# lucadellalib/audiocodecs

Measured on AMD Instinct MI355X. Metric: encode+decode audio-sec/s, EnCodec-24k 8cb, higher is better.
Workload: dtype f32 (GEMM-shaped kernels and LSTM products: operands as two scaled fp16 planes, 3 partial products, fp32 accumulate -- split16.h)

## Files before the change

### audiocodecs_amd/csrc/ac_api.hip

```cpp
#include "core.h"
#include "tap_route.h"

extern "C" {

int ac_version(void) { return 400; }

int ac_create(const ac_config* cfg, ac_handle** out) {
    if (!cfg || !out) return AC_EINVAL;
    *out = nullptr;
    if (cfg->struct_size != (int32_t)sizeof(ac_config)) return AC_EINVAL;
    if (cfg->num_ratios < 1 || cfg->num_ratios > AC_MAX_RATIOS || cfg->num_filters < 1 || cfg->hidden_size < 16 ||
        cfg->hidden_size % 16 || cfg->compress < 1 || cfg->num_lstm_layers < 1 || cfg->num_lstm_layers > 2 || cfg->codebook_size % 32 ||
        cfg->codebook_size < 16 || cfg->num_quantizers < 1 || cfg->kernel_size < 1 || cfg->kernel_size > 8 ||
        cfg->last_kernel_size < 1 || cfg->last_kernel_size > 8 || cfg->residual_kernel_size < 1 || cfg->residual_kernel_size > 8)
        return AC_EINVAL;
    int ndev = 0;
    if (hipGetDeviceCount(&ndev) != hipSuccess || ndev <= cfg->device || cfg->device < 0) return AC_ENODEV;
    ac_handle* h = new (std::nothrow) ac_handle();
    if (!h) return AC_ENOMEM;
    h->cfg = *cfg;
    h->hop = 1;
    for (int i = 0; i < cfg->num_ratios; ++i) h->hop *= cfg->upsampling_ratios[i];
    h->D = cfg->num_filters << cfg->num_ratios;
    *out = h;
    return AC_OK;
}







static std::string wavtok_key(const std::string& name) {
    static const std::string pre = "feature_extractor.encodec.encoder.model.";
    if (name.compare(0, pre.size(), pre) != 0) return name;
    std::string k = "encoder.layers." + name.substr(pre.size());
    const size_t cc = k.find(".conv.conv.");
    if (cc != std::string::npos) k = k.substr(0, cc) + ".conv." + k.substr(cc + 11);
    auto ends = [&](const char* sfx) { const size_t n = std::strlen(sfx); return k.size() >= n && k.compare(k.size() - n, n, sfx) == 0; };
    if (ends(".weight_g")) k = k.substr(0, k.size() - 9) + ".parametrizations.weight.original0";
    else if (ends(".weight_v")) k = k.substr(0, k.size() - 9) + ".parametrizations.weight.original1";
    return k;
}

int ac_load_weights(ac_handle* h, const char* name, const void* host_ptr, size_t bytes) {
    if (!h || !name || !host_ptr) return h ? fail(h, AC_EINVAL, "null argument") : AC_EINVAL;
    if (h->finalized) return fail(h, AC_ESTATE, "handle already finalized");
    if (bytes % 4) return fail(h, AC_EINVAL, "tensor '%s': byte size %zu is not a multiple of 4", name, bytes);
    const float* f = static_cast<const float*>(host_ptr);
    h->host[h->arch == ARCH_WAVTOK ? wavtok_key(name) : std::string(name)].assign(f, f + bytes / 4);
    return AC_OK;
}



static void latch_dev_switches(ac_handle* h) {
    auto num = [](const char* name, int dflt) { const char* v = std::getenv(name); return v && *v ? std::atoi(v) : dflt; };
    const char* e = std::getenv("AC_TAP_EPI");
    h->dev.tap_epi_staged = e && std::strcmp(e, "staged") == 0;
    h->dev.tap_dil = num("AC_TAP_DIL", 1);
    h->dev.tap_stagger = num("AC_TAP_STAGGER", 0);
    h->dev.tap_pick = num("AC_TAP_PICK", -1);
    h->dev.tap8 = num("AC_TAP8", -1);
    h->dev.tap8_form = num("AC_TAP8_FORM", 0);
    h->dev.tap8_spread = num("AC_TAP8_SPREAD", 1);
#ifdef AC_DEVELOPER
    h->dev.rb6_dbg = num("AC_RB6_DBG", 0);
    h->dev.lstm_dbg = num("AC_LSTM_DBG", 0);
#endif
    h->dev.rb_stream = num("AC_RB_STREAM", 1);
    h->dev.chain_stream = num("AC_CHAIN_STREAM", 1);
    h->dev.rb128_stream = num("AC_RB128_STREAM", 1);
    h->dev.rb256_fused = num("AC_RB256_FUSED", 1);
    h->dev.front_seg = std::max(0, num("AC_FRONT_SEG", 0));
    h->dev.tail_seg = std::max(0, num("AC_TAIL_SEG", 0));
    h->dev.front_ldspad = std::max(0, num("AC_FRONT_LDSPAD", 0));
    h->dev.lstm_fuse_in = num("AC_LSTM_FUSE_IN", 1);
    const char* r = std::getenv("AC_RVQ");
    h->dev.rvq_exact = r && std::strcmp(r, "fp32") == 0;
    h->dev.prof_detail = num("AC_PROF_DETAIL", 0);
    h->dev.head_seq = num("AC_HEAD_SEQ", 0);
    h->dev.attn_exact = num("AC_ATTN_EXACT", 0);
    h->dev.dac_unit = num("AC_DAC_UNIT", 1);
    h->dev.mimi_tail = num("AC_MIMI_TAIL", 1);
    h->dev.mstream_skinny = num("AC_MSTREAM_SKINNY", -1);
}

int ac_debug_set(ac_handle* h, const char* key, int value) {
    if (!h || !key) return AC_EINVAL;
    struct { const char* k; int* v; } tab[] = {
        {"tap_epi_staged", &h->dev.tap_epi_staged}, {"tap_dil", &h->dev.tap_dil}, {"tap_stagger", &h->dev.tap_stagger}, {"tap_pick", &h->dev.tap_pick}, {"tap8", &h->dev.tap8}, {"tap8_form", &h->dev.tap8_form}, {"tap8_spread", &h->dev.tap8_spread},
        {"rb6_dbg", &h->dev.rb6_dbg}, {"rb_stream", &h->dev.rb_stream}, {"chain_stream", &h->dev.chain_stream}, {"rb128_stream", &h->dev.rb128_stream}, {"rb256_fused", &h->dev.rb256_fused}, {"front_seg", &h->dev.front_seg}, {"tail_seg", &h->dev.tail_seg}, {"front_ldspad", &h->dev.front_ldspad},
        {"lstm_dbg", &h->dev.lstm_dbg}, {"lstm_fuse_in", &h->dev.lstm_fuse_in}, {"rvq_exact", &h->dev.rvq_exact}, {"prof_detail", &h->dev.prof_detail}, {"head_seq", &h->dev.head_seq}, {"attn_exact", &h->dev.attn_exact}, {"dac_unit", &h->dev.dac_unit}, {"mimi_tail", &h->dev.mimi_tail},
        {"mstream_skinny", &h->dev.mstream_skinny},
    };
#ifndef AC_DEVELOPER
    if (std::strcmp(key, "rb6_dbg") == 0 || std::strcmp(key, "lstm_dbg") == 0)
        return fail(h, AC_EINVAL, "ac_debug_set('%s'): a developer-build switch (timing modes with wrong results / fault injection); this is the product library", key);
#endif
    if (!h->finalized) return fail(h, AC_ESTATE, "ac_debug_set('%s'): the switches are latched by ac_finalize; set them afterwards", key);
    for (auto& t : tab)
        if (std::strcmp(t.k, key) == 0) {
            const bool nonneg = t.v == &h->dev.front_seg || t.v == &h->dev.tail_seg || t.v == &h->dev.front_ldspad || t.v == &h->dev.tap_stagger;
            if (nonneg && value < 0) return fail(h, AC_EINVAL, "ac_debug_set('%s', %d): the value must be >= 0", key, value);
            if (t.v == &h->dev.front_ldspad && value > 16384) return fail(h, AC_EINVAL, "ac_debug_set('front_ldspad', %d): at most 16384 bytes", value);
            if (t.v == &h->dev.tap8_form && (value < 0 || value > 5)) return fail(h, AC_EINVAL, "ac_debug_set('tap8_form', %d): 0 (cost model) .. 5", value);
            *t.v = value;
            return AC_OK;
        }
    return fail(h, AC_EINVAL, "ac_debug_set: unknown switch '%s'", key);
}

int ac_set_precision(ac_handle* h, int precision) {
    if (!h) return AC_EINVAL;
    if (h->finalized) return fail(h, AC_ESTATE, "ac_set_precision must precede ac_finalize (weights are packed for one arithmetic)");
    if (precision != AC_PRECISION_FP32 && precision != AC_PRECISION_FP32_EXACT) return fail(h, AC_EINVAL, "unknown precision %d", precision);
    h->precision = precision;
    return AC_OK;
}

int ac_finalize(ac_handle* h) {
    if (!h) return AC_EINVAL;
    if (h->finalized) return fail(h, AC_ESTATE, "handle already finalized");
    {
        int pr = h->precision;
        if (pr < 0) {
            const char* gm = std::getenv("AC_GEMM");
            if (gm && *gm && std::strcmp(gm, "fp32") != 0 && std::strcmp(gm, "split16") != 0)
                return fail(h, AC_EINVAL, "AC_GEMM=%s: unknown arithmetic (fp32 = exact fp32 products, split16 or unset = the default)", gm);
            pr = gm && std::strcmp(gm, "fp32") == 0 ? AC_PRECISION_FP32_EXACT : AC_PRECISION_FP32;
        }
        const char* fz = std::getenv("AC_FUSE");
        h->fuse_chains = !(fz && fz[0] == '0');
        latch_dev_switches(h);
        h->gemm_fp32 = pr == AC_PRECISION_FP32_EXACT;
    }
    if (h->arch == ARCH_MIMI) {
        Packer pk{h};
        if (int rc = mimi_finalize(h, pk)) return rc;
        return upload_blob(h, pk, h->mcfg.device);
    }
    if (h->arch == ARCH_DAC) {
        Packer pk{h};
        if (int rc = dac_finalize(h, pk)) return rc;
        return upload_blob(h, pk, h->dcfg.device);
    }
    if (h->arch == ARCH_WAVTOK) {
        Packer pk{h};
        if (int rc = wavtok_finalize(h, pk)) return rc;
        return upload_blob(h, pk, h->wcfg.device);
    }
    const ac_config& c = h->cfg;
    Arch a = make_arch(c);
    Packer pk{h};
    h->has_enc = h->has_dec = false;
    for (const auto& kv : h->host) {
        if (kv.first.compare(0, 8, "encoder.") == 0) h->has_enc = true;
        if (kv.first.compare(0, 8, "decoder.") == 0) h->has_dec = true;
    }
    if (!h->has_enc && !h->has_dec) return fail(h, AC_ESTATE, "no encoder.* or decoder.* tensor was loaded");
    bool ok = true;
    h->enc_rb.resize(c.num_ratios);
    h->enc_down.resize(c.num_ratios);
    h->dec_up.resize(c.num_ratios);
    h->dec_rb.resize(c.num_ratios);
    if (h->has_enc) {
        ok = pk.conv(a.enc_stem, h->enc_stem);
        for (int i = 0; ok && i < c.num_ratios; ++i) {
            ok = ok && pk.resblock(a.enc_rb3[i], a.enc_rb1[i], a.enc_rbs[i], h->enc_rb[i]);
            ok = ok && pk.conv(a.enc_down[i], h->enc_down[i]);
        }
        ok = ok && pk.lstm(a.enc_lstm, a.D, c.num_lstm_layers, h->enc_lstm);
        ok = ok && pk.conv(a.enc_final, h->enc_final);
        if (ok) pk.chain_bounds(h->enc_stem, h->enc_rb[0], h->enc_down[0], h->enc_front);
// ... 577 lines not shown
```

### audiocodecs_amd/csrc/core.h

```cpp
#pragma once
#include <hip/hip_runtime.h>

#include <algorithm>
#include <cmath>
#include <cstdarg>
#include <cstdio>
#include <cstdlib>
#include <cstring>
#include <map>
#include <string>
#include <vector>

#include "../../include/audiocodecs_amd.h"
#include "lstm_consts.h"
#include "rvq_types.h"
#include "split16.h"
#include "tap_gemm.h"

using namespace ac;

namespace ac {
constexpr int THIN_MAXK = 8;
struct RbFused6Params;
}

namespace acimpl {


struct ConvSpec {
    std::string prefix;
    int transposed, cin, cout, k, s;
};

struct PackedGemm {
    size_t w_off = 0, b_off = 0;
    int N = 0, Ktot = 0;
    bool has_bias = true;
};

struct ResBlockPlan {
    int C;
    PackedGemm c3;
    PackedGemm fused;
    size_t w3f_off = 0, wff_off = 0;
    size_t winv3_off = 0, winvf_off = 0;
    size_t w3p_off = 0, wfp_off = 0;
    float hb0 = 0.f, hb1 = 0.f;
    bool has6 = false;
    bool hb256 = false;
};

struct LstmPlan {
    int D, layers;
    std::vector<PackedGemm> ih;
    std::vector<size_t> hh_off;
    std::vector<size_t> ihpk_off;
    size_t persist_off = 0;
    size_t persist16_off = 0;
    size_t persist16_inv = 0;
    bool has_persist = false;
};

struct MimiTfLayer {
    PackedGemm qkv, o, fc1, fc2;
    size_t ln1_w = 0, ln1_b = 0, ln2_w = 0, ln2_b = 0, sc_a = 0, sc_m = 0;
};

struct MimiPlan {
    PackedGemm enc_stem, enc_final, down, dec_first, dec_head;
    std::vector<ResBlockPlan> enc_rb, dec_rb;
    std::vector<PackedGemm> enc_down, dec_up;
    std::vector<MimiTfLayer> enc_tf, dec_tf;
    size_t up_w = 0;
    PackedGemm in_proj;
    PackedGemm out_proj;
    size_t cb_plain = 0, cb_packed = 0, cb_ee = 0;
    size_t cb16 = 0, cb16_inv = 0;
    size_t rope_cos = 0, rope_sin = 0;
    int rope_T = 0;
    int D = 0;
    struct StreamM { size_t stem_f = 0, stem_inv = 0, head_f = 0, head_inv = 0; float sb0 = 0.f, sb1 = 0.f, fb0 = 0.f, fb1h = 0.f; bool stem_ok = false, head_ok = false; } sm;
};

struct DacResUnitPlan {
    PackedGemm c7, c1;
    size_t a1 = 0, a1i = 0, a2 = 0, a2i = 0;
    int dil = 1;
};

struct DacBlockPlan {
    int C = 0, stride = 1;
    std::vector<DacResUnitPlan> ru;
    size_t a = 0, ai = 0;
    PackedGemm conv;
};

struct DacPlan {
    PackedGemm enc_stem, enc_final, dec_first, dec_head, in_proj0;
    std::vector<DacBlockPlan> enc, dec;
    size_t enc_a = 0, enc_ai = 0, dec_a = 0, dec_ai = 0;
    size_t win = 0, bin = 0, wout = 0, bout = 0, cb = 0, cbn = 0, c2 = 0, proj = 0;
    int H = 0;
};

struct WtResnetPlan {
    size_t n1w = 0, n1b = 0, n2w = 0, n2b = 0;
    PackedGemm c1, c2;
};
struct WtCnxPlan {
    size_t dww = 0, dwb = 0, sc = 0, sh = 0, gamma = 0;
    PackedGemm p1, p2;
};
struct WavtokPlan {
    PackedGemm embed, qkv, proj, head, istft;
    WtResnetPlan rn[4];
    size_t an_w = 0, an_b = 0;
    size_t g5w = 0, g5b = 0;
    size_t nsc = 0, nsh = 0;
    size_t flw = 0, flb = 0;
    size_t w2 = 0;
    std::vector<WtCnxPlan> cnx;
    int bins = 0, npad = 0, hop_pad = 0, taps = 0;
};

struct ProfRec {
    int name_id;
    int count;
    hipEvent_t e0, e1;
    double flops, bytes;
};


}
using namespace acimpl;

enum { ARCH_ENCODEC = 0, ARCH_MIMI = 1, ARCH_DAC = 2, ARCH_WAVTOK = 3 };

struct ac_handle {
    int arch = ARCH_ENCODEC;
    ac_config cfg{};
    ac_mimi_config mcfg{};
    MimiPlan mimi;
    ac_dac_config dcfg{};
    DacPlan dac;
    ac_wavtok_config wcfg{};
    WavtokPlan wt;
    std::string err;
    std::map<std::string, std::vector<float>> host;
    bool finalized = false;
    float* blob = nullptr;
    size_t blob_floats = 0;
    int hop = 1, D = 0;
    PackedGemm enc_stem, enc_final;
    std::vector<ResBlockPlan> enc_rb;
    std::vector<PackedGemm> enc_down;
    LstmPlan enc_lstm, dec_lstm;
    PackedGemm dec_first, dec_head;
    std::vector<PackedGemm> dec_up;
    std::vector<ResBlockPlan> dec_rb;
    size_t cb_plain = 0, cb_packed = 0, cb_ee = 0;
    size_t cb16 = 0, cb16_inv = 0;
    struct ChainBounds { float sb0 = 0.f, sb1 = 0.f, fb0 = 0.f, fb1h = 0.f, fb1x = 0.f; bool ok = false; } enc_front, dec_tail;
    struct StreamImgs { size_t stem_f = 0, stem_inv = 0, down_f = 0, down_inv = 0, up_f = 0, up_inv = 0, head_f = 0, head_inv = 0; bool enc_ok = false, dec_ok = false; } simg;
    struct DevSwitches {
        int tap_epi_staged = 0;
        int tap_dil = 1;
        int tap_stagger = 0;
        int tap_pick = -1;
        int tap8 = -1;
        int tap8_form = 0;
        int tap8_spread = 1;
        int rb6_dbg = 0;
        int rb_stream = 1;
        int rb256_fused = 1;
        int rb128_stream = 1;
        int chain_stream = 1;
        int front_seg = 0, tail_seg = 0;
        int front_ldspad = 0;
        int lstm_dbg = 0;
        int lstm_fuse_in = 1;
        int rvq_exact = 0;
        int prof_detail = 0;
        int attn_exact = 0;
        int dac_unit = 1;
        int mimi_tail = 1;
        int head_seq = 0;
        int mstream_skinny = -1;
    } dev;
    bool fuse_chains = true;
    float* dbg = nullptr;
    size_t dbg_cap = 0, dbg_used = 0;
    std::vector<const void*> lds_opted;
    std::map<size_t, size_t> w6_of;
    std::map<size_t, size_t> t6_of;
    std::map<size_t, size_t> t6inv_of;
    bool noncausal = false;
    bool has_enc = true, has_dec = true;
    bool gemm_fp32 = false;
    std::map<size_t, size_t> winv_of;
    std::map<const void*, int> mimi_streams;
    std::map<const void*, int> mimi_dstreams;
    struct EStreamReg {
        int B;
        std::vector<uint8_t> fresh;
    };
    std::map<const void*, EStreamReg> encodec_streams, encodec_dstreams;
    unsigned* amax_buf = nullptr;
    int amax_B = 0, amax_next = 0;
    unsigned* row_buf = nullptr;
    size_t row_cap = 0, row_next = 0;
    void* own_pool = nullptr;
    size_t own_pool_rows = 0;
    int precision = -1;
    unsigned* lp_ctl = nullptr;
    int num_cus = 0;
    bool lstm_step_only = false;
    unsigned long long* clk_dev = nullptr;
    unsigned* sticky = nullptr;
    unsigned* sticky_dev = nullptr;
    bool prof = false;
    bool prof_detail = false;
    std::vector<ProfRec> recs;
    std::vector<std::string> prof_names;
    std::vector<hipEvent_t> ev_pool;
    size_t ev_used = 0;
};

namespace acimpl {

int fail(ac_handle* h, int code, const char* fmt, ...);


#define HIPCHK(h, call)                                                                         \
    do {                                                                                        \
        hipError_t e_ = (call);                                                                 \
        if (e_ != hipSuccess) return fail(h, AC_EHIP, "%s failed: %s", #call, hipGetErrorString(e_)); \
    } while (0)


inline int cdiv(int a, int b) { return (a + b - 1) / b; }

int ensure_lds(ac_handle* h, const void* func, size_t bytes);

inline size_t align_up(size_t v, size_t a) { return (v + a - 1) / a * a; }


struct Arch {
    std::vector<ConvSpec> enc_rb3, enc_rb1, enc_rbs, enc_down;
    ConvSpec enc_stem, enc_final, dec_first, dec_head;
    std::vector<ConvSpec> dec_up, dec_rb3, dec_rb1, dec_rbs;
    std::string enc_lstm, dec_lstm;
    int D;
};

Arch make_arch(const ac_config& c);


struct Packer {
    ac_handle* h;
    std::vector<float> blob;
    int rc = AC_OK;

    const std::vector<float>* get(const std::string& name, size_t n) {
        auto it = h->host.find(name);
        if (it == h->host.end()) {
            rc = fail(h, AC_ESTATE, "missing tensor '%s'", name.c_str());
            return nullptr;
        }
        if (it->second.size() != n) {
            rc = fail(h, AC_EINVAL, "tensor '%s' has %zu elements, expected %zu", name.c_str(), it->second.size(), n);
            return nullptr;
        }
        return &it->second;
    }
    bool weight(const ConvSpec& s, std::vector<float>& w) {
        const size_t n = (size_t)s.cin * s.cout * s.k;
        auto it = h->host.find(s.prefix + ".weight");
        if (it != h->host.end()) {
            if (it->second.size() != n) {
                rc = fail(h, AC_EINVAL, "tensor '%s.weight' has %zu elements, expected %zu", s.prefix.c_str(), it->second.size(), n);
                return false;
// ... 345 lines not shown
    void tail_bounds(const PackedGemm& up, const ResBlockPlan& rb, const PackedGemm& head, ac_handle::ChainBounds& cb) {
        cb.ok = false;
        if (!use16() || !rb.has6 || !rb.winv3_off || rb.C != 32 || up.N != 64 || up.Ktot != 128 || !h->t6inv_of.count(up.w_off) || head.N != 1 || head.Ktot != 7 * 32) return;
        cb.sb0 = cb.sb1 = 0.f;
        for (int n = 0; n < up.N; ++n) {
            double l1 = 0.0;
            for (int k = 0; k < up.Ktot; ++k) l1 += std::fabs((double)blob[up.w_off + (size_t)n * up.Ktot + k]);
            cb.sb1 = std::max(cb.sb1, (float)(l1 * 1.000001));
            cb.sb0 = std::max(cb.sb0, std::fabs(blob[up.b_off + n]));
        }
        const int hid = rb.C / 2;
        cb.fb0 = cb.fb1h = cb.fb1x = 0.f;
        for (int n = 0; n < rb.C; ++n) {
            double lh = 0.0, lx = 0.0;
            for (int k = 0; k < hid; ++k) lh += std::fabs((double)blob[rb.fused.w_off + (size_t)n * rb.fused.Ktot + k]);
            for (int k = hid; k < rb.fused.Ktot; ++k) lx += std::fabs((double)blob[rb.fused.w_off + (size_t)n * rb.fused.Ktot + k]);
            cb.fb1h = std::max(cb.fb1h, (float)(lh * 1.000001));
            cb.fb1x = std::max(cb.fb1x, (float)(lx * 1.000001));
            cb.fb0 = std::max(cb.fb0, std::fabs(blob[rb.fused.b_off + n]));
        }
        cb.ok = true;
    }
    bool lstm(const std::string& prefix, int D, int layers, LstmPlan& lp) {
        lp.D = D;
        lp.layers = layers;
        for (int l = 0; l < layers; ++l) {
            const std::string sfx = "_l" + std::to_string(l);
            const std::vector<float>* wih = get(prefix + ".weight_ih" + sfx, (size_t)4 * D * D);
            const std::vector<float>* whh = get(prefix + ".weight_hh" + sfx, (size_t)4 * D * D);
            const std::vector<float>* bih = get(prefix + ".bias_ih" + sfx, (size_t)4 * D);
            const std::vector<float>* bhh = get(prefix + ".bias_hh" + sfx, (size_t)4 * D);
            if (!wih || !whh || !bih || !bhh) return false;
            PackedGemm g;
            g.N = 4 * D;
            g.Ktot = D;
            g.w_off = reserve((size_t)4 * D * D);
            std::copy(wih->begin(), wih->end(), blob.begin() + g.w_off);
            g.b_off = reserve((size_t)4 * D);
            for (int n = 0; n < 4 * D; ++n) blob[g.b_off + n] = (*bih)[n] + (*bhh)[n];
            if (l == 0) pack6(g);
            lp.ih.push_back(g);
            const size_t off = reserve((size_t)4 * D * D);
            for (int ug = 0; ug < D / 4; ++ug)
                for (int ks = 0; ks < D / 16; ++ks)
                    for (int lane = 0; lane < 64; ++lane)
                        for (int u = 0; u < 4; ++u) {
                            const int j = lane & 15, kq = lane >> 4;
                            const int row = (j >> 2) * D + ug * 4 + (j & 3);
                            const int k = ks * 16 + 4 * kq + u;
                            blob[off + (((size_t)ug * (D / 16) + ks) * 64 + lane) * 4 + u] = (*whh)[(size_t)row * D + k];
                        }
            lp.hh_off.push_back(off);
            const size_t off2 = reserve((size_t)4 * D * D);
            for (int ug = 0; ug < D / 4; ++ug)
                for (int ks = 0; ks < D / 16; ++ks)
                    for (int lane = 0; lane < 64; ++lane)
                        for (int u = 0; u < 4; ++u) {
                            const int j = lane & 15, kq = lane >> 4;
                            const int row = (j >> 2) * D + ug * 4 + (j & 3);
                            const int k = ks * 16 + 4 * kq + u;
                            blob[off2 + (((size_t)ug * (D / 16) + ks) * 64 + lane) * 4 + u] = (*wih)[(size_t)row * D + k];
                        }
            lp.ihpk_off.push_back(off2);
        }
        if (D == LP_D && layers == 2) {
            const std::vector<float>* mats[3] = {get(prefix + ".weight_hh_l0", (size_t)4 * D * D), get(prefix + ".weight_ih_l1", (size_t)4 * D * D),
                                                 get(prefix + ".weight_hh_l1", (size_t)4 * D * D)};
            const size_t mat = (size_t)LP_SLICES * 4 * 4 * 8 * 256;
            lp.persist_off = reserve(3 * mat);
            for (int m = 0; m < 3; ++m)
                for (int idx = 0; idx < LP_SLICES; ++idx)
                    for (int w = 0; w < 4; ++w)
                        for (int n = 0; n < 4; ++n)
                            for (int ks = 0; ks < 8; ++ks)
                                for (int lane = 0; lane < 64; ++lane)
                                    for (int e = 0; e < 4; ++e)
                                        blob[lp.persist_off + m * mat + ((((size_t)idx * 4 + w) * 4 + n) * 8 + ks) * 256 + lane * 4 + e] =
                                            (*mats[m])[(size_t)(n * D + idx * 16 + (lane & 15)) * D + (w * 8 + ks) * 16 + 4 * (lane >> 4) + e];
            const std::vector<float>* mats6[4] = {mats[0], mats[1], mats[2], get(prefix + ".weight_ih_l0", (size_t)4 * D * D)};
            if (use16()) {
                const size_t mat16 = (size_t)LP_SLICES * 4 * 4 * 4 * 2 * 512;
                lp.persist16_off = reserve((4 * mat16 + 1) / 2);
                lp.persist16_inv = reserve((size_t)2 * 4 * D);
                std::vector<int> sc((size_t)2 * 4 * D);
                const int layer_of[4] = {0, 1, 1, 0};
                for (int l = 0; l < 2; ++l)
                    for (int row = 0; row < 4 * D; ++row) {
                        uint32_t mx = 0;
                        for (int m = 0; m < 4; ++m)
                            if (layer_of[m] == l)
                                for (int k = 0; k < D; ++k) {
                                    uint32_t b;
                                    std::memcpy(&b, &(*mats6[m])[(size_t)row * D + k], 4);
                                    mx = std::max(mx, b & 0x7fffffffu);
                                }
                        sc[(size_t)l * 4 * D + row] = s16_exponent(mx, 40);
                        blob[lp.persist16_inv + (size_t)l * 4 * D + row] = s16_pow2(-sc[(size_t)l * 4 * D + row]);
                    }
                std::vector<uint16_t> pl16(4 * mat16);
                for (int m = 0; m < 4; ++m)
                    for (int idx = 0; idx < LP_SLICES; ++idx)
                        for (int w = 0; w < 4; ++w)
                            for (int n = 0; n < 4; ++n)
                                for (int ks = 0; ks < 4; ++ks)
                                    for (int lane = 0; lane < 64; ++lane)
                                        for (int e = 0; e < 8; ++e) {
                                            const int row = n * D + idx * 16 + (lane & 15);
                                            uint16_t t[3];
                                            split16h((*mats6[m])[(size_t)row * D + w * 128 + ks * 32 + 8 * (lane >> 4) + e], sc[(size_t)layer_of[m] * 4 * D + row], t);
                                            const size_t base = m * mat16 + (((((size_t)idx * 4 + w) * 4 + n) * 4 + ks) * 2) * 512 + (size_t)lane * 8 + e;
                                            pl16[base] = t[0];
                                            pl16[base + 512] = t[1];
                                        }
                std::memcpy(&blob[lp.persist16_off], pl16.data(), pl16.size() * 2);
            }
            lp.has_persist = true;
        }
        return true;
    }
};


struct Act {
    const float* p;
    long long bs, ts;
    int L, C;
    const unsigned* amax = nullptr;
    int amax_n = 0;
};

int prof_name(ac_handle* h, const char* nm);

hipEvent_t next_event(ac_handle* h);


struct ProfScope {
    ac_handle* h;
    hipStream_t st;
    ProfRec r{};
    bool on;
    ProfScope(ac_handle* h_, hipStream_t st_, const char* nm, double flops, double bytes, int count = 1)
        : h(h_), st(st_), on(h_->prof) {
        if (!on) return;
        r.name_id = prof_name(h, nm);
        r.count = count;
        r.flops = flops;
        r.bytes = bytes;
        r.e0 = next_event(h);
        r.e1 = next_event(h);
        (void)hipEventRecord(r.e0, st);
    }
    ~ProfScope() {
        if (!on) return;
        (void)hipEventRecord(r.e1, st);
        h->recs.push_back(r);
    }
};


constexpr int AMAX_SLOTS = 512;

inline size_t pool_bytes(int pool_B, size_t rows) {
    return (size_t)AMAX_SLOTS * std::max(pool_B, 1) * AMAX_STRIDE * 4 + 8 * align_up(std::max<size_t>(rows, 64), 64) * 4 + 256;
}

void pool_bind(ac_handle* h, void* mem, int pool_B, size_t rows);

int amax_begin(ac_handle* h, hipStream_t st, int B);

unsigned* amax_new(ac_handle* h);

const unsigned* amax_of(ac_handle* h, hipStream_t st, const float* x, long long bs, long long ts, int L, int C, int B, const unsigned* known);

unsigned* rowmax_new(ac_handle* h, hipStream_t st, long long rows, bool zero);

const unsigned* amax_plus(ac_handle* h, hipStream_t st, const Act& x, float add, int B);

TapSeg make_seg(const Act& x, int s, int J, int pad , int extra, int kofs, const float* rel_len, int left = -1, int right = 0);


inline bool aligned16(const void* p) { return (reinterpret_cast<uintptr_t>(p) & 15) == 0; }

int run_tap(ac_handle* h, hipStream_t st, TapGemmParams& p);


struct Out {
    float* raw = nullptr;
    float* elu = nullptr;
};

struct Act2 {
    Act raw{}, elu{};
};

int try_thin6(ac_handle* h, hipStream_t st, const PackedGemm& g, const Act& x, int width, int edge, Out out, int B, const unsigned** amax_out = nullptr);

int conv_fwd(ac_handle* h, hipStream_t st, const PackedGemm& g, const Act& x, int k, int s, const float* rel_len, Out out,
             long long out_bs, long long out_rs, int B, Act2* y);

int convtr_fwd(ac_handle* h, hipStream_t st, const PackedGemm& g, const Act& x, int s, Out out, int B, Act2* y);

bool rb128_ok(const ac_handle* h, const ResBlockPlan& rb);

int resblock_fwd(ac_handle* h, hipStream_t st, const ResBlockPlan& rb, const Act2& x, float* hbuf, Out out, int B, Act2* y);
bool rb256_ok(const ac_handle* h, const ResBlockPlan& rb, int L);

bool thin_ok(const ac_config& c, int k);

int thin_stem(ac_handle* h, hipStream_t st, const PackedGemm& g, int F, int k, int pad, const float* sig, const float* rel_len, int B, int T,
              Out out, Act2* y, int padl = -1, const float* alpha = nullptr, const float* alpha_inv = nullptr, int Lp = -1);

int stem_fwd(ac_handle* h, hipStream_t st, const float* sig, const float* rel_len, int B, int T, Out out, Act2* y);

int thin_head(ac_handle* h, hipStream_t st, const PackedGemm& g, int F, int k, int pad, const Act& x, int B, float* sig, int padl = -1,
              int tanh_out = 0);

int head_fwd(ac_handle* h, hipStream_t st, const Act& x, int B, float* sig);

bool enc_front_ok(const ac_handle* h, int T);

int enc_front_fwd(ac_handle* h, hipStream_t st, const float* sig, const float* rel_len, int B, int T, float* y, float* dbg_x0, float* dbg_y1, Act2* out);

bool dec_tail_ok(const ac_handle* h, const Act& xe);

int dec_tail_fwd(ac_handle* h, hipStream_t st, const Act& xe, int B, float* sig, float* dbg_u, float* dbg_v);

void capture(ac_handle* h, hipStream_t st, const Act& a, int B);


struct LstmWs {
    float *gin, *gin1, *hseq0, *hseq1, *c;
};

int lstm_fwd(ac_handle* h, hipStream_t st, const LstmPlan& lp, const Act& x, const LstmWs& ws, Out out, int B, Act2* y);

int rvq_encode_fwd(ac_handle* h, hipStream_t st, const float* feats, int F, int K, long long* toks);

int rvq_decode_fwd(ac_handle* h, hipStream_t st, const long long* toks, int F, int K, float* out);


constexpr int NACT = 6;


struct Workspace {
    size_t act_floats = 0;
    size_t gin = 0, hseq = 0, c = 0;
    int pool_B = 0;
    size_t pool_rows = 0;
    size_t total_bytes = 0;
};

inline void add_pool(Workspace& w, int pool_B, size_t rows) {
    w.pool_B = pool_B;
    w.pool_rows = rows;
    w.total_bytes += pool_bytes(pool_B, rows);
}

Workspace plan_ws(const ac_handle* h, int B, int T_in , int N_frames , bool enc);


struct WsPtrs {
    float* act[NACT];
    bool used[NACT];
    LstmWs lstm;
    float* take() {
        for (int i = 0; i < NACT; ++i)
            if (!used[i]) { used[i] = true; return act[i]; }
        return nullptr;
    }
    void give(const float* p) {
        for (int i = 0; i < NACT; ++i)
            if (act[i] == p) used[i] = false;
    }
    void give(const Act2& a) { give(a.raw.p); give(a.elu.p); }
};

int carve(ac_handle* h, const Workspace& w, void* ws, size_t ws_bytes, WsPtrs* o);

int check_ready(ac_handle* h);

int check_len(ac_handle* h, long long samples);

int encoder_fwd(ac_handle* h, hipStream_t st, const float* sig, const float* rel_len, int B, int T, float* feats, WsPtrs& ws);

int decoder_fwd(ac_handle* h, hipStream_t st, const long long* toks, int B, int N, int K, float* sig, WsPtrs& ws);

bool rb64_identity_head_fwd(ac_handle* h, hipStream_t st, const ResBlockPlan& rb, const Act2& x, const PackedGemm& head, int head_k, float* sig, int B, int* rc);
int enc_stream_fwd(ac_handle* h, hipStream_t st, const float* sig, const float* rel_len, int B, int T, float* y, float* dbg_x0, float* dbg_y1, const unsigned* amax_sig, unsigned* amax_out);
int dec_stream_fwd(ac_handle* h, hipStream_t st, const Act& xe, int B, float* sig, float* dbg_u, float* dbg_v, const unsigned* amax_x);
int launch_rb_stream6m(ac_handle* h, hipStream_t st, const ResBlockPlan& rb, const float* xr, const float* sig, int B, int L, Out out, float* head_y, int head_k,
                       const unsigned* amax_in, unsigned* amax_out);
int launch_rb_stream128m(ac_handle* h, hipStream_t st, RbFused6Params& p, const ResBlockPlan& rb, bool sc, Out out, int B);
int launch_rb_stream6(ac_handle* h, hipStream_t st, RbFused6Params& p, const ResBlockPlan& rb, bool sc, Out out, int B);
int rb64_identity_fwd(ac_handle* h, hipStream_t st, const ResBlockPlan& rb, const Act2& x, Out out, int B, const unsigned** amax_out);
int rb128_identity_fwd(ac_handle* h, hipStream_t st, const ResBlockPlan& rb, const Act2& x, Out out, int B, const unsigned** amax_out);
int rvq_encode_cdist_launch(ac_handle* h, hipStream_t st, const RvqEncParams& p, unsigned blocks, const _Float16* epk16 = nullptr, const float* einv = nullptr);
void rvq_decode_launch(hipStream_t st, const RvqDecParams& p, unsigned blocks);
void amax_fill_launch(hipStream_t st, unsigned* slot, unsigned bits, int B);
int resample_launch(const float* x, int B, int L, const float* kern, int n, int o, int taps, int width, float* y, int L_out, hipStream_t st);
constexpr int RSTREAM_MAX_TAPS = 8192;
long long resample_stream_groups(long long total, int o, int width);
long long resample_stream_out_len(long long consumed, int L, int n, int o, int width, int finish);
size_t resample_stream_state_bytes(int B, int taps);
int resample_stream_reset_launch(void* state, int B, int n, int o, int taps, int width, hipStream_t st);
int resample_stream_push_launch(void* state, const float* x, long long x_pitch, int B, int L, long long consumed, const float* kern, int n, int o, int taps,
                                int width, float* y, long long y_pitch, int m, int finish, hipStream_t st);
int resample_stream_reset_slots_launch(void* state, int B, int n, int o, int taps, int width, const int* slots_dev, int rows, hipStream_t st);
int resample_stream_push_slots_launch(void* state, int B, const int* slots_dev, const long long* consumed_dev, int rows, const float* x, long long x_pitch,
                                      int L, const float* kern, int n, int o, int taps, int width, float* y, long long y_pitch, int m, int finish,
                                      hipStream_t st);

struct Epi {
    const float* scale = nullptr;
    const float* res = nullptr;
    long long res_bs = 0, res_rs = 0;
    int gelu = 0;
    const unsigned* rowmax_in = nullptr;
// ... 32 lines not shown
```

### audiocodecs_amd/csrc/core.hip

```cpp
#include "core.h"
#include "split16_kernels.h"
#include "lstm.h"
#include "lstm_persist.h"
#include "lstm_persist16.h"
#include "rvq.h"
#include "rvq16.h"
#include "tap_gemm4.h"
#include "tap_gemm6.h"
#include "tap_gemm8.h"
#include "tap_route.h"
#include "thin.h"
#include "rb_fused.h"
#include "rb_fused6.h"
#include "thin_conv6.h"
#include "rb_fused6_128.h"
#include "rb256_fused.h"
#include "enc_front.h"
#include "dec_tail.h"

namespace acimpl {


int fail(ac_handle* h, int code, const char* fmt, ...) {
    char buf[1024];
// ... 126 lines not shown
        zero_words(st, r, need);
        if (hipGetLastError() != hipSuccess) return nullptr;
    }
    return r;
}


const unsigned* amax_plus(ac_handle* h, hipStream_t st, const Act& x, float add, int B) {
    if (!x.amax || x.amax_n != B) return nullptr;
    unsigned* slot = amax_new(h);
    if (!slot) return nullptr;
    hipLaunchKernelGGL(amax_add_kernel, dim3(cdiv(B, 64)), dim3(64), 0, st, x.amax, add, slot, B);
    return slot;
}



template <int WGM, int WGN, int WM, int WN>
static int launch_tap(ac_handle* h, hipStream_t st, TapGemmParams p, TapFamily f, const char* name, double flops, double bytes) {
    ProfScope ps(h, st, name, flops, bytes);
    if (f == TapFamily::tap4) {
        using Cfg = Tap4Cfg<WGM, WGN, WM, WN>;
        p.mtiles = cdiv(p.M, Cfg::BM);
        p.ntiles = cdiv(p.N, Cfg::BN);
        if (int rc = ensure_lds(h, reinterpret_cast<const void*>(tap_gemm4_kernel<WGM, WGN, WM, WN>), Cfg::lds_bytes)) return rc;
        const long long blocks = (long long)p.B * p.mtiles * p.ntiles;
        hipLaunchKernelGGL((tap_gemm4_kernel<WGM, WGN, WM, WN>), dim3((unsigned)blocks), dim3(Cfg::NT), Cfg::lds_bytes, st, p);
        return AC_OK;
    }
    constexpr int BM = WGM * WM * 16, BN = WGN * WN * 16;
    p.mtiles = cdiv(p.M, BM);
    p.ntiles = cdiv(p.N, BN);
    const size_t lds = tap_gemm_lds_bytes<WGM, WGN, WM, WN>();
    const long long blocks = (long long)p.B * p.mtiles * p.ntiles;
    if (f == TapFamily::vec) hipLaunchKernelGGL((tap_gemm_kernel<WGM, WGN, WM, WN, true>), dim3((unsigned)blocks), dim3(WGM * WGN * 64), lds, st, p);
    else hipLaunchKernelGGL((tap_gemm_kernel<WGM, WGN, WM, WN, false>), dim3((unsigned)blocks), dim3(WGM * WGN * 64), lds, st, p);
    return AC_OK;
}

static int launch_tap_fp32(ac_handle* h, hipStream_t st, const TapGemmParams& p, const TapRoute& r, const char* name, double flops, double bytes) {
    switch (r.key()) {
    case tap_key(4, 1, 2, 1): return launch_tap<4, 1, 2, 1>(h, st, p, r.family, name, flops, bytes);
    case tap_key(4, 1, 2, 2): return launch_tap<4, 1, 2, 2>(h, st, p, r.family, name, flops, bytes);
    case tap_key(2, 2, 2, 2): return launch_tap<2, 2, 2, 2>(h, st, p, r.family, name, flops, bytes);
    case tap_key(2, 2, 4, 3): return launch_tap<2, 2, 4, 3>(h, st, p, r.family, name, flops, bytes);
    case tap_key(2, 2, 4, 4): return launch_tap<2, 2, 4, 4>(h, st, p, r.family, name, flops, bytes);
    }
    return fail(h, AC_EINVAL, "run_tap: no instantiation of %s", r.name);
}

template <int WGM, int WGN, int WMT, int WN, int HALO>
static int launch_tap6(ac_handle* h, hipStream_t st, TapGemmParams& p, const __bf16* w6, const char* name, double flops, double bytes) {
    using Cfg = Tap6Cfg<WGM, WGN, WMT, WN, HALO>;
    p.mtiles = cdiv(p.M, Cfg::BM);
    p.ntiles = p.N / Cfg::BN;
    const long long blocks = (long long)p.B * p.mtiles * p.ntiles;
    if (int rc = ensure_lds(h, reinterpret_cast<const void*>(tap_gemm6_kernel<WGM, WGN, WMT, WN, 2, HALO>), Cfg::lds_for(2))) return rc;
    ProfScope ps(h, st, name, flops, bytes);
    hipLaunchKernelGGL((tap_gemm6_kernel<WGM, WGN, WMT, WN, 2, HALO>), dim3((unsigned)blocks), dim3(Cfg::NT), Cfg::lds_for(2), st, p, w6);
    return AC_OK;
}

static int launch_tap6_family(ac_handle* h, hipStream_t st, TapGemmParams& p, const TapRoute& r, const __bf16* w6, const char* name, double flops, double bytes) {
    if (r.family == TapFamily::tap6_dil) {
        switch (r.key()) {
        case tap_key(1, 4, 4, 2): return launch_tap6<1, 4, 4, 2, T6_DIL_HALO>(h, st, p, w6, name, flops, bytes);
        case tap_key(1, 4, 4, 1): return launch_tap6<1, 4, 4, 1, T6_DIL_HALO>(h, st, p, w6, name, flops, bytes);
        case tap_key(2, 2, 2, 3): return launch_tap6<2, 2, 2, 3, T6_DIL_HALO>(h, st, p, w6, name, flops, bytes);
        case tap_key(4, 1, 1, 3): return launch_tap6<4, 1, 1, 3, T6_DIL_HALO>(h, st, p, w6, name, flops, bytes);
        }
    } else {
        switch (r.key()) {
        case tap_key(1, 4, 4, 2): return launch_tap6<1, 4, 4, 2, 7>(h, st, p, w6, name, flops, bytes);
        case tap_key(1, 8, 4, 1): return launch_tap6<1, 8, 4, 1, 7>(h, st, p, w6, name, flops, bytes);
        case tap_key(1, 4, 4, 1): return launch_tap6<1, 4, 4, 1, 7>(h, st, p, w6, name, flops, bytes);
        case tap_key(2, 2, 2, 3): return launch_tap6<2, 2, 2, 3, 7>(h, st, p, w6, name, flops, bytes);
        case tap_key(4, 1, 1, 3): return launch_tap6<4, 1, 1, 3, 7>(h, st, p, w6, name, flops, bytes);
        case tap_key(2, 2, 2, 1): return launch_tap6<2, 2, 2, 1, 7>(h, st, p, w6, name, flops, bytes);
        }
    }
    return fail(h, AC_EINVAL, "run_tap: no instantiation of %s", r.name);
}

template <int WGM, int WGN, int WMT, int WN, bool RM, bool J1, bool SP>
static int launch_tap8(ac_handle* h, hipStream_t st, TapGemmParams& p, const __bf16* w6, const char* name, double flops, double bytes) {
    using Cfg = Tap8Cfg<WGM, WGN, WMT, WN>;
    p.mtiles = cdiv(p.M, Cfg::BM);
    p.ntiles = p.N / Cfg::BN;
    const long long blocks = (long long)p.B * p.mtiles * p.ntiles;
    ProfScope ps(h, st, name, flops, bytes);
    if (int rc = ensure_lds(h, reinterpret_cast<const void*>(tap_gemm8_kernel<WGM, WGN, WMT, WN, RM, J1, SP>), Cfg::lds_bytes)) return rc;
    hipLaunchKernelGGL((tap_gemm8_kernel<WGM, WGN, WMT, WN, RM, J1, SP>), dim3((unsigned)blocks), dim3(Cfg::NT), Cfg::lds_bytes, st, p, w6);
    return AC_OK;
}

static int launch_tap8_family(ac_handle* h, hipStream_t st, TapGemmParams& p, const TapRoute& r, const __bf16* w6, const char* name, double flops, double bytes) {
    constexpr int RJ = TK_RM | TK_J1, J = TK_J1, S = TK_SPREAD;
    switch (r.key()) {
    case tap_key(2, 4, 4, 2, RJ): return launch_tap8<2, 4, 4, 2, true, true, false>(h, st, p, w6, name, flops, bytes);
    case tap_key(2, 4, 4, 2, RJ | S): return launch_tap8<2, 4, 4, 2, true, true, true>(h, st, p, w6, name, flops, bytes);
    case tap_key(2, 4, 4, 2, J): return launch_tap8<2, 4, 4, 2, false, true, false>(h, st, p, w6, name, flops, bytes);
    case tap_key(2, 4, 4, 2, J | S): return launch_tap8<2, 4, 4, 2, false, true, true>(h, st, p, w6, name, flops, bytes);
    case tap_key(2, 4, 4, 2): return launch_tap8<2, 4, 4, 2, false, false, false>(h, st, p, w6, name, flops, bytes);
    case tap_key(2, 4, 4, 2, S): return launch_tap8<2, 4, 4, 2, false, false, true>(h, st, p, w6, name, flops, bytes);
    case tap_key(2, 4, 2, 2, RJ): return launch_tap8<2, 4, 2, 2, true, true, false>(h, st, p, w6, name, flops, bytes);
    case tap_key(2, 4, 2, 2, RJ | S): return launch_tap8<2, 4, 2, 2, true, true, true>(h, st, p, w6, name, flops, bytes);
    case tap_key(2, 4, 2, 2, J): return launch_tap8<2, 4, 2, 2, false, true, false>(h, st, p, w6, name, flops, bytes);
    case tap_key(2, 4, 2, 2, J | S): return launch_tap8<2, 4, 2, 2, false, true, true>(h, st, p, w6, name, flops, bytes);
    case tap_key(2, 4, 2, 2): return launch_tap8<2, 4, 2, 2, false, false, false>(h, st, p, w6, name, flops, bytes);
    case tap_key(2, 4, 2, 2, S): return launch_tap8<2, 4, 2, 2, false, false, true>(h, st, p, w6, name, flops, bytes);
    case tap_key(4, 2, 2, 2, RJ): return launch_tap8<4, 2, 2, 2, true, true, false>(h, st, p, w6, name, flops, bytes);
    case tap_key(4, 2, 2, 2, RJ | S): return launch_tap8<4, 2, 2, 2, true, true, true>(h, st, p, w6, name, flops, bytes);
    case tap_key(4, 2, 2, 2, J): return launch_tap8<4, 2, 2, 2, false, true, false>(h, st, p, w6, name, flops, bytes);
    case tap_key(4, 2, 2, 2, J | S): return launch_tap8<4, 2, 2, 2, false, true, true>(h, st, p, w6, name, flops, bytes);
    case tap_key(4, 2, 2, 2): return launch_tap8<4, 2, 2, 2, false, false, false>(h, st, p, w6, name, flops, bytes);
    case tap_key(4, 2, 2, 2, S): return launch_tap8<4, 2, 2, 2, false, false, true>(h, st, p, w6, name, flops, bytes);
    }
    return fail(h, AC_EINVAL, "run_tap: no instantiation of %s", r.name);
}


TapSeg make_seg(const Act& x, int s, int J, int pad , int extra, int kofs, const float* rel_len, int left, int right) {
    TapSeg g{};
    g.x = x.p;
    g.amax = x.amax;
    g.amax_n = x.amax_n;
    g.bs = x.bs;
    g.ts = x.ts;
    g.rel_len = rel_len;
    g.L = x.L;
    g.cin = x.C;
    g.cin_shift = -1;
    for (int sh = 0; sh < 30; ++sh)
        if ((1 << sh) == x.C) g.cin_shift = sh;
    g.s = s;
    g.J = J;
    const int pad_left = left < 0 ? (J - 1) * s : left;
    const int max_pad = std::max(pad_left, right + extra);
    g.Lp = (pad == PAD_REFLECT && x.L <= max_pad) ? max_pad + 1 : x.L;
    g.lim = pad != PAD_ZERO ? x.L + right + extra : x.L;
    g.reflect = pad;
    g.elu = 0;
    g.kofs = kofs;
    g.pad = pad_left;
    g.dil = 1;
    return g;
}


int run_tap(ac_handle* h, hipStream_t st, TapGemmParams& p) {
    const auto w6_it = h->w6_of.find((size_t)(p.w - h->blob));
    const auto iv = h->winv_of.find((size_t)(p.w - h->blob));
    TapRouteInputs in;
    in.w6 = w6_it != h->w6_of.end();
    in.winv = iv != h->winv_of.end();
    in.want_rowmode = p.amax_rows != 0;
    in.want_rows = p.amax_out_rows != nullptr;
    in.gemm_fp32 = h->gemm_fp32;
    const TapRoute r = route_tap(p, in, h->dev);
    if (r.reject_taps) return fail(h, AC_EINVAL, "conv with %d taps exceeds the kernel limit of 8", r.reject_taps);
    double kk = 0, inb = 0;
    for (int i = 0; i < p.nseg; ++i) {
        kk += (double)p.seg[i].J * p.seg[i].s * p.seg[i].cin;
        inb += (double)p.B * p.seg[i].L * p.seg[i].cin * 4.0;
    }
    const double flops = 2.0 * p.B * (double)p.M * p.N * kk;
    const double bytes = inb + (double)p.B * p.M * p.N * 4.0 * ((p.y ? 1 : 0) + (p.y_elu ? 1 : 0)) + (double)p.N * p.Ktot * 4.0;
    std::string name = r.name;
    if (h->prof && h->prof_detail && r.family != TapFamily::scalar && r.family != TapFamily::vec) {
        char shape[64];
        std::snprintf(shape, sizeof shape, " B%d M%d N%d K%d J%d s%d%s", p.B, p.M, p.N, (int)kk, p.seg[0].J, p.seg[0].s, p.seg[0].dil == 1 ? "" : p.seg[0].dil == 3 ? " d3" : " d9");
        name += shape;
    }
    p.amax_out_rows = nullptr;
    p.amax_rows = 0;
    int rc;
    if (r.family == TapFamily::scalar || r.family == TapFamily::vec || r.family == TapFamily::tap4) {
        rc = launch_tap_fp32(h, st, p, r, name.c_str(), flops, bytes);
    } else {
        p.clk = h->clk_dev;
#ifdef T6_TRACE
        if (const char* ts = std::getenv("AC_TRACE_SHAPE")) {
            int tm = 0, tn = 0, tk = 0;
            if (std::sscanf(ts, "%d,%d,%d", &tm, &tn, &tk) == 3 && !((tm == 0 || tm == p.M) && tn == p.N && tk == (int)kk)) p.clk = nullptr;
        }
#endif
        if (r.rowmode) {
            TapSeg& sg = p.seg[0];
            if (!(sg.amax && sg.amax_n == -p.M)) {
                unsigned* rm = rowmax_new(h, st, p.M, false);
                if (!rm) return fail(h, AC_ENOMEM, "the workspace pool's row ring is too small for %d rows", p.M);
                ProfScope ps(h, st, "rowmax_kernel", 0.0, (double)p.M * sg.cin * 4.0);
                hipLaunchKernelGGL(rowmax_kernel, dim3((unsigned)cdiv(p.M, 4)), dim3(256), 0, st, sg.x, sg.ts, (long long)p.M, sg.cin, rm);
                sg.amax = rm;
            }
            p.amax_rows = 1;
            p.winv = h->blob + iv->second;
            if (r.rows_out) {
                p.amax_out_rows = rowmax_new(h, st, p.M, true);
                if (!p.amax_out_rows) return fail(h, AC_ENOMEM, "the workspace pool's row ring is too small for %d rows", p.M);
            }
        } else if (in.winv) {
            for (int i = 0; i < p.nseg; ++i) {
                TapSeg& sg = p.seg[i];
                sg.amax = amax_of(h, st, sg.x, sg.bs, sg.ts, sg.L, sg.cin, p.B, sg.amax_n == p.B ? sg.amax : nullptr);
                if (!sg.amax) return fail(h, AC_ESTATE, "out of amax slots (split16.h)");
            }
            p.winv = h->blob + iv->second;
            p.amax_out = amax_new(h);
            p.epi_direct = r.epi_direct;
        }
        p.stagger = h->dev.tap_stagger;
        const __bf16* w6 = reinterpret_cast<const __bf16*>(h->blob + w6_it->second);
        rc = r.family == TapFamily::tap8 ? launch_tap8_family(h, st, p, r, w6, name.c_str(), flops, bytes)
                                         : launch_tap6_family(h, st, p, r, w6, name.c_str(), flops, bytes);
    }
    if (rc) return rc;
    HIPCHK(h, hipGetLastError());
    return AC_OK;
}


int try_thin6(ac_handle* h, hipStream_t st, const PackedGemm& g, const Act& x, int width, int edge, Out out, int B, const unsigned** amax_out) {
    if (h->gemm_fp32 || g.N != 64 || g.Ktot != 128 || x.C != width || x.ts != width || x.bs != (long long)x.L * width ||
        (x.L * width) % 64 || x.L * width < 256 || !aligned16(x.p) || (long long)x.L * width * 4 > 0x70000000LL)
        return 1;
    auto it = h->t6_of.find(g.w_off);
    if (it == h->t6_of.end()) return 1;
    ThinConv6Params p{};
    p.x = x.p;
    p.wf = reinterpret_cast<const __bf16*>(h->blob + it->second);
    p.bias = h->blob + g.b_off;
    p.y = out.raw;
    p.y_elu = out.elu;
    p.B = B;
    p.Ls = x.L * width / 64;
    p.M = p.Ls;
    p.ntiles = cdiv(p.M, T6_BM);
    p.edge = edge;
    const bool s16 = h->t6inv_of.count(g.w_off) != 0;
    if (s16) {
        p.amax_in = amax_of(h, st, x.p, x.bs, x.ts, x.L, x.C, B, x.amax_n == B ? x.amax : nullptr);
        if (!p.amax_in) return fail(h, AC_ESTATE, "out of amax slots (split16.h)");
        p.winv = h->blob + h->t6inv_of[g.w_off];
        p.amax_out = amax_new(h);
        if (amax_out) *amax_out = p.amax_out;
    }
    const long long total = (long long)B * p.ntiles;
    const int grid = (int)std::min<long long>(total, 4 * 256);
    ProfScope ps(h, st, "thin_conv6_kernel<2>", 2.0 * B * p.M * 64.0 * 128.0,
                 (double)B * p.M * 256.0 * (1 + (out.raw ? 1 : 0) + (out.elu ? 1 : 0)));
    hipLaunchKernelGGL(thin_conv6_kernel<2>, dim3(grid), dim3(256), T6_LDS, st, p);
    return AC_OK;
}


int conv_fwd(ac_handle* h, hipStream_t st, const PackedGemm& g, const Act& x, int k, int s, const float* rel_len, Out out,
             long long out_bs, long long out_rs, int B, Act2* y) {
    const int M = cdiv(x.L, s);
    const int extra = M * s - x.L;
    if (s == 2 && k == 4 && !rel_len && extra == 0 && x.L >= 4 && out_rs == 64 && out_bs == (long long)M * 64 && !h->noncausal) {
        const unsigned* am = nullptr;
        const int rc = try_thin6(h, st, g, x, 32, 1, out, B, &am);
        if (rc <= 0) {
            if (y && !rc) {
                y->raw = Act{out.raw, out_bs, out_rs, M, g.N, am, B};
                y->elu = Act{out.elu, out_bs, out_rs, M, g.N, am, B};
            }
            if (!rc) HIPCHK(h, hipGetLastError());
            return rc;
        }
    }
    TapGemmParams p{};
    p.nseg = 1;
    if (s != 1 && k != 2 * s) return fail(h, AC_EINVAL, "strided conv needs kernel == 2*stride (got k=%d, s=%d)", k, s);
    if (h->noncausal) {
        const int total = k - s, right = total / 2;
        p.seg[0] = make_seg(x, s, s == 1 ? k : 2, PAD_REFLECT, extra, 0, rel_len, total - right, right);
    } else {
        p.seg[0] = make_seg(x, s, s == 1 ? k : 2, PAD_REFLECT, extra, 0, rel_len);
    }
    p.w = h->blob + g.w_off;
    p.bias = g.has_bias ? h->blob + g.b_off : nullptr;
    p.y = out.raw;
    p.y_elu = out.elu;
    p.y_bs = out_bs;
    p.y_rs = out_rs;
    p.B = B;
    p.M = M;
    p.N = g.N;
    p.Ktot = g.Ktot;
    const int rc = run_tap(h, st, p);
    if (y) {
        y->raw = Act{out.raw, out_bs, out_rs, M, g.N, p.amax_out, p.B};
        y->elu = Act{out.elu, out_bs, out_rs, M, g.N, p.amax_out, p.B};
    }
    return rc;
}


int convtr_fwd(ac_handle* h, hipStream_t st, const PackedGemm& g, const Act& x, int s, Out out, int B, Act2* y) {
    const int cout = g.N / s;
    if (s == 2) {
        const unsigned* am = nullptr;
        const int rc = try_thin6(h, st, g, x, 64, 0, out, B, &am);
        if (rc <= 0) {
            if (!rc) {
                y->raw = Act{out.raw, (long long)x.L * s * cout, cout, x.L * s, cout, am, B};
                y->elu = Act{out.elu, (long long)x.L * s * cout, cout, x.L * s, cout, am, B};
                HIPCHK(h, hipGetLastError());
            }
            return rc;
        }
    }
    TapGemmParams p{};
    p.nseg = 1;
    p.seg[0] = make_seg(x, 1, 2, PAD_ZERO, 0, 0, nullptr);
    p.w = h->blob + g.w_off;
    p.bias = h->blob + g.b_off;
    p.y = out.raw;
    p.y_elu = out.elu;
    p.y_bs = (long long)x.L * g.N;
    p.y_rs = g.N;
    p.B = B;
    p.M = x.L;
    p.N = g.N;
    p.Ktot = g.Ktot;
    const int rc = run_tap(h, st, p);
    y->raw = Act{out.raw, (long long)x.L * s * cout, cout, x.L * s, cout, p.amax_out, p.B};
    y->elu = Act{out.elu, (long long)x.L * s * cout, cout, x.L * s, cout, p.amax_out, p.B};
    return rc;
}


template <int C, int BM, int NSPLIT, bool SC = true>
int launch_rb_fused(ac_handle* h, hipStream_t st, const ResBlockPlan& rb, const Act2& x, Out out, int B, int pad = PAD_REFLECT) {
    using Cfg = RbCfg<C, BM, NSPLIT, SC>;
    RbFusedParams p{};
    p.xe = x.elu.p;
    p.xr = x.raw.p;
    p.w3 = h->blob + rb.c3.w_off;
    p.b3 = h->blob + rb.c3.b_off;
    p.wf = h->blob + rb.fused.w_off;
    p.bf = h->blob + rb.fused.b_off;
    p.y = out.raw;
    p.y_elu = out.elu;
    p.B = B;
    p.L = x.raw.L;
    p.Lp = x.raw.L > 2 ? x.raw.L : 3;
    p.ntiles = cdiv(x.raw.L, BM);
    p.pad = pad;
    if (int rc = ensure_lds(h, reinterpret_cast<const void*>(rb_fused_kernel<C, BM, NSPLIT, SC>), Cfg::lds_bytes)) return rc;
    const long long total = (long long)B * p.ntiles;
    const int grid = (int)std::min<long long>(total, 512);
    const size_t lds = Cfg::lds_bytes;
    const double L = x.raw.L;
    ProfScope ps(h, st, !SC ? "rb_fused_kernel<64, 64, 2, false>" : C == 32 ? "rb_fused_kernel<32, 128, 1>" : "rb_fused_kernel<64, 64, 2>",
                 2.0 * B * L * ((double)(C / 2) * 3 * C + (double)C * Cfg::KF),
                 (double)B * L * C * 4.0 * ((x.elu.p ? 2 : 1) + (out.raw ? 1 : 0) + (out.elu ? 1 : 0)));
    hipLaunchKernelGGL((rb_fused_kernel<C, BM, NSPLIT, SC>), dim3(grid), dim3(256), lds, st, p);
    return AC_OK;
}


bool rb_split16(ac_handle* h, hipStream_t st, const ResBlockPlan& rb, const Act2& x, int B, RbFused6Params& p, const unsigned** amax_out) {
    if (h->gemm_fp32 || !rb.winv3_off) return false;
    p.amax_in = amax_of(h, st, x.raw.p, x.raw.bs, x.raw.ts, x.raw.L, x.raw.C, B, x.raw.amax_n == B ? x.raw.amax : nullptr);
    p.winv3 = h->blob + rb.winv3_off;
    p.winvf = h->blob + rb.winvf_off;
    p.hb0 = rb.hb0;
    p.hb1 = rb.hb1;
    p.amax_out = amax_new(h);
    if (amax_out) *amax_out = p.amax_out;
    return true;
}


template <int C, bool SC>
int launch_rb_fused6(ac_handle* h, hipStream_t st, const ResBlockPlan& rb, const Act2& x, Out out, int B, int pad = PAD_REFLECT, const unsigned** amax_out = nullptr,
                     const PackedGemm* head = nullptr, int head_k = 0, float* head_y = nullptr) {
    using Cfg = Rb6Cfg<C, SC>;
    RbFused6Params p{};
    const bool with_head = head && C == 64 && !SC;
    if (with_head) {
        p.head_w = h->blob + head->w_off;
        p.head_b = h->blob + head->b_off;
        p.head_y = head_y;
        p.head_k = head_k;
    }
    p.xr = x.raw.p;
    p.w3f = reinterpret_cast<const __bf16*>(h->blob + rb.w3f_off);
    p.wff = reinterpret_cast<const __bf16*>(h->blob + rb.wff_off);
    p.b3 = h->blob + rb.c3.b_off;
    p.bf = h->blob + rb.fused.b_off;
    p.y = out.raw;
    p.y_elu = out.elu;
    p.B = B;
    p.L = x.raw.L;
    p.lpad = h->noncausal ? 1 : 2;
    p.Lp = x.raw.L > p.lpad ? x.raw.L : p.lpad + 1;
    p.ntiles = cdiv(x.raw.L, with_head ? Cfg::BM - (head_k - 1) : Cfg::BM);
    p.pad = pad;
    p.dbg = h->dev.rb6_dbg;
    if (!rb_split16(h, st, rb, x, B, p, amax_out)) return fail(h, AC_ESTATE, "fused residual block without split16 images");
    if (!p.amax_in) return fail(h, AC_ESTATE, "out of amax slots (split16.h)");
    if (with_head) p.amax_out = nullptr;
    const double L = x.raw.L;
    if (C == 64 && !with_head && h->dev.rb_stream && p.lpad == 2 && rb.w3p_off && (long long)x.raw.L * 256 < 0x70000000LL)
        return launch_rb_stream6(h, st, p, rb, SC, out, B);
    const size_t lds6 = with_head ? Cfg::lds_bytes16_head : Cfg::lds_bytes16;
// ... 295 lines not shown
        return AC_OK;
    }
    size_t lds = EF_LDS;
    lds += (size_t)h->dev.front_ldspad;
    if (int rc = ensure_lds(h, reinterpret_cast<const void*>(enc_front_kernel), lds)) return rc;
    const long long streams = (long long)B * p.segs_per_clip;
    {
        ProfScope ps(h, st, "enc_front_kernel", 2.0 * B * (double)T * (7.0 * 32 + 16.0 * 96 + 32.0 * 48 + 64.0 * 128 / 2),
                     (double)B * T * 4.0 + (double)B * p.M * 256.0);
        hipLaunchKernelGGL(enc_front_kernel, dim3((unsigned)cdiv((int)streams, EF_WAVES)), dim3(64 * EF_WAVES), lds, st, p);
    }
    HIPCHK(h, hipGetLastError());
    out->raw = Act{y, (long long)p.M * 64, 64, p.M, 64, p.amax_out, B};
    out->elu = Act{nullptr, (long long)p.M * 64, 64, p.M, 64, p.amax_out, B};
    return AC_OK;
}


bool dec_tail_ok(const ac_handle* h, const Act& xe) {
    const ac_config& c = h->cfg;
    return h->fuse_chains && h->arch == ARCH_ENCODEC && !h->noncausal && !h->gemm_fp32 && h->dec_tail.ok &&
           c.num_filters == 32 && c.last_kernel_size == 7 && c.residual_kernel_size == 3 && c.compress == 2 && c.num_ratios >= 1 &&
           c.upsampling_ratios[c.num_ratios - 1] == 2 && xe.p && xe.C == 64 && xe.ts == 64 && xe.bs == (long long)xe.L * 64 && aligned16(xe.p) &&
           xe.L >= 32 && (long long)xe.L * 256 < 0x70000000LL;
}


int dec_tail_fwd(ac_handle* h, hipStream_t st, const Act& xe, int B, float* sig, float* dbg_u, float* dbg_v) {
    const int last = h->cfg.num_ratios - 1;
    const ResBlockPlan& rb = h->dec_rb[last];
    const PackedGemm& gu = h->dec_up[last];
    DecTailParams p{};
    p.xe = xe.p;
    p.wuf = reinterpret_cast<const __bf16*>(h->blob + h->t6_of[gu.w_off]);
    p.w3f = reinterpret_cast<const __bf16*>(h->blob + rb.w3f_off);
    p.wff = reinterpret_cast<const __bf16*>(h->blob + rb.wff_off);
    p.bu = h->blob + gu.b_off;
    p.winvu = h->blob + h->t6inv_of[gu.w_off];
    p.b3 = h->blob + rb.c3.b_off;
    p.winv3 = h->blob + rb.winv3_off;
    p.bf = h->blob + rb.fused.b_off;
    p.winvf = h->blob + rb.winvf_off;
    p.wh = h->blob + h->dec_head.w_off;
    p.bh = h->blob + h->dec_head.b_off;
    p.sig = sig;
    p.dbg_u = dbg_u;
    p.dbg_v = dbg_v;
    p.B = B;
    p.L = xe.L;
    const int nchunks = cdiv(xe.L, DT_ROWS);
    p.seg_chunks = std::max(8, cdiv(nchunks, std::max(1, 6144 / B)));
    if (h->dev.tail_seg > 0) p.seg_chunks = h->dev.tail_seg;
    p.segs_per_clip = cdiv(nchunks, p.seg_chunks);
    p.amax_x = amax_of(h, st, xe.p, xe.bs, xe.ts, xe.L, xe.C, B, xe.amax_n == B ? xe.amax : nullptr);
    if (!p.amax_x) return fail(h, AC_ESTATE, "out of amax slots (split16.h)");
    p.ub0 = h->dec_tail.sb0; p.ub1 = h->dec_tail.sb1;
    p.hb0 = rb.hb0; p.hb1 = rb.hb1;
    if (h->dev.chain_stream && h->simg.dec_ok) {
        if (int rc = dec_stream_fwd(h, st, xe, B, sig, dbg_u, dbg_v, p.amax_x)) return rc;
        HIPCHK(h, hipGetLastError());
        return AC_OK;
    }
    if (int rc = ensure_lds(h, reinterpret_cast<const void*>(dec_tail_kernel), DT_LDS)) return rc;
    const long long streams = (long long)B * p.segs_per_clip;
    {
        ProfScope ps(h, st, "dec_tail_kernel", 2.0 * B * (double)xe.L * (64.0 * 128 + 2.0 * (16.0 * 96 + 32.0 * 48 + 7.0 * 32)),
                     (double)B * xe.L * 256.0 + (double)B * xe.L * 8.0);
        hipLaunchKernelGGL(dec_tail_kernel, dim3((unsigned)cdiv((int)streams, 8)), dim3(512), DT_LDS, st, p);
    }
    HIPCHK(h, hipGetLastError());
    return AC_OK;
}


void capture(ac_handle* h, hipStream_t st, const Act& a, int B) {
    if (!h->dbg) return;
    const size_t n = (size_t)B * a.L * a.C;
    if (h->dbg_used + n <= h->dbg_cap)
        (void)hipMemcpyAsync(h->dbg + h->dbg_used, a.p, n * sizeof(float), hipMemcpyDeviceToDevice, st);
    h->dbg_used += n;
}


int lstm_fwd(ac_handle* h, hipStream_t st, const LstmPlan& lp, const Act& x, const LstmWs& ws, Out out, int B, Act2* y) {
    const int D = lp.D, T = x.L, L = lp.layers;
    if (D % 64 != 0 || D > 512) return fail(h, AC_EINVAL, "LSTM width %d unsupported (need 64, 128, 256 or 512)", D);
    if (L < 1 || L > 2) return fail(h, AC_EINVAL, "%d LSTM layers unsupported (1 or 2)", L);
    hipStreamCaptureStatus cap = hipStreamCaptureStatusNone;
    (void)hipStreamIsCapturing(st, &cap);
    const bool persist = lp.has_persist && h->lp_ctl && h->num_cus == 256 && !h->lstm_step_only && x.ts == D && cap == hipStreamCaptureStatusNone;
    const bool fuse_env = h->dev.lstm_fuse_in != 0;
    const bool fuse_in = persist && !h->gemm_fp32 && fuse_env && aligned16(x.p) && x.bs % 4 == 0;
    if (!fuse_in) {
        TapGemmParams p{};
        p.nseg = 1;
        p.seg[0] = make_seg(x, 1, 1, PAD_ZERO, 0, 0, nullptr);
        p.w = h->blob + lp.ih[0].w_off;
        p.bias = h->blob + lp.ih[0].b_off;
        p.y = ws.gin;
        p.y_bs = 4LL * D;
        p.y_rs = (long long)B * 4 * D;
        p.B = B;
        p.M = T;
        p.N = 4 * D;
        p.Ktot = D;
        int rc = run_tap(h, st, p);
        if (rc) return rc;
    }
    const int nroles = 2 * L - 1, nlaunch = T + 2 * (L - 1);
    const long long BD = (long long)((B + 31) / 32 * 32) * D, B4D = (long long)B * 4 * D;
    if (persist) {
        const int chunks = cdiv(B, 64);
        const unsigned* x_amax = nullptr;
        if (fuse_in && lp.persist16_inv) {
            x_amax = amax_of(h, st, x.p, x.bs, x.ts, x.L, x.C, B, x.amax_n == B ? x.amax : nullptr);
            if (!x_amax) return fail(h, AC_ESTATE, "out of amax slots (split16.h)");
        }
        int* poison = reinterpret_cast<int*>(ws.c);
        if (!h->gemm_fp32) HIPCHK(h, hipMemsetAsync(poison, 0x7f, (size_t)B * sizeof(int), st));
        ProfScope ps(h, st, h->gemm_fp32 ? "lstm_persist_kernel" : fuse_in ? "lstm_persist16_kernel<true>" : "lstm_persist16_kernel<false>", 2.0 * T * (double)B * 4 * D * D * (nroles + (fuse_in ? 1 : 0)),
                     (double)T * ((double)B * 4 * D * 4 + 3.0 * B * D * 4) + 12.0 * D * D * 4, chunks);
        auto tail = [&](int c0, int nb, const int* pz) {
            LstmTailParams tp{};
            tp.ctl = h->lp_ctl;
            tp.sticky = h->sticky_dev;
            tp.poison = pz;
            tp.yout = out.raw;
            tp.yout_elu = out.elu;
            tp.y_bs = (long long)T * D;
            tp.clip0 = c0;
            tp.B = nb;
            tp.T = T;
            tp.D = D;
            tp.xcds_used = 8;
            hipLaunchKernelGGL(lstm_tail_kernel, dim3(nb, 4), dim3(256), 0, st, tp);
        };
        for (int c0 = 0; c0 < B; c0 += 64) {
            LstmPersistParams q{};
            q.gin0 = ws.gin;
            q.w_pk = h->blob + lp.persist_off;
            q.bias1 = h->blob + lp.ih[1].b_off;
            q.hseq0 = ws.hseq0;
            q.hseq1 = ws.hseq1;
            q.skip = x.p;
            q.yout = out.raw;
            q.yout_elu = out.elu;
            q.ctl = h->lp_ctl;
            q.gin_ts = B4D;
            q.h_ts = BD;
            q.skip_bs = x.bs;
            q.y_bs = (long long)T * D;
            q.B = std::min(64, B - c0);
            q.T = T;
            q.group0 = c0 / 16;
            q.clip0 = c0;
            q.dbg = h->dev.lstm_dbg;
            if (!h->gemm_fp32) {
                LstmPersist16Params q6{};
                q6.base = q;
                q6.base.h_ts = (long long)((B + 31) / 32 * 2) * LP16_GROUP_BYTES;
                q6.winv = h->blob + lp.persist16_inv;
                q6.amax_x = fuse_in ? x_amax : nullptr;
                q6.w_pk6 = reinterpret_cast<const __bf16*>(h->blob + lp.persist16_off);
                q6.bias0 = h->blob + lp.ih[0].b_off;
                q6.fuse_in = fuse_in ? 1 : 0;
                q6.poison = poison;
                q6.hseq0_local = ws.gin1;
                HIPCHK(h, hipMemsetAsync(h->lp_ctl, 0, LP_CTL_WORDS * sizeof(unsigned), st));
                const size_t hbytes = (size_t)T * (size_t)q6.base.h_ts;
                const size_t rbytes = (size_t)std::min(T, LP16_RING) * (size_t)q6.base.h_ts;
                HIPCHK(h, hipMemsetAsync(ws.hseq0, 0xFF, hbytes, st));
                HIPCHK(h, hipMemsetAsync(ws.hseq1, 0xFF, rbytes, st));
                HIPCHK(h, hipMemsetAsync(ws.gin1, 0xFF, rbytes, st));
                void* args6[] = {&q6};
                const void* kfn = fuse_in ? reinterpret_cast<const void*>(lstm_persist16_kernel<true>) : reinterpret_cast<const void*>(lstm_persist16_kernel<false>);
                HIPCHK(h, hipLaunchCooperativeKernel(kfn, dim3(256), dim3(512), args6, 0, st));
                tail(c0, q.B, poison);
                if (AC_DEV_MODE(q.dbg, 32)) {
                    HIPCHK(h, hipStreamSynchronize(st));
                    std::vector<unsigned long long> tr(8 * 64);
                    HIPCHK(h, hipMemcpy(tr.data(), h->lp_ctl + LP_CTL_FLAGS, tr.size() * 8, hipMemcpyDeviceToHost));
                    for (int role = 0; role < 2; ++role) {
                        std::fprintf(stderr, "lstm trace role %d (layer %d), 10 ns units from step start: ", role, role & 1);
                        for (int s_ = 0; s_ < 4; ++s_) {
                            const unsigned long long* r = &tr[role * 64 + s_ * 8];
                            std::fprintf(stderr, "| t=%d:", 100 + s_);
                            for (int k = 1; k < 8; ++k) std::fprintf(stderr, " %lld", r[k] ? (long long)(r[k] - r[0]) : -1LL);
                            if (s_ < 3) std::fprintf(stderr, " next %lld ", (long long)(r[8] - r[0]));
                        }
                        const double us3 = (double)(tr[role * 64 + 24] - tr[role * 64]) * 0.01;
                        std::fprintf(stderr, " | steps that had to poll: %llu of %d | shader clock %.0f MHz\n", tr[role * 64 + 63], T,
                                     us3 > 0 ? (double)(tr[role * 64 + 33] - tr[role * 64 + 32]) / us3 : 0.0);
                    }
                }
                continue;
            }
            HIPCHK(h, hipMemsetAsync(h->lp_ctl, 0, LP_CTL_WORDS * sizeof(unsigned), st));
            void* args[] = {&q};
            HIPCHK(h, hipLaunchCooperativeKernel(reinterpret_cast<const void*>(lstm_persist_kernel), dim3(256), dim3(256), args, 0, st));
            tail(c0, q.B, nullptr);
        }
        HIPCHK(h, hipGetLastError());
        const unsigned* am = amax_plus(h, st, x, 1.0f, B);
        y->raw = Act{out.raw, (long long)T * D, D, T, D, am, B};
        y->elu = Act{out.elu, (long long)T * D, D, T, D, am, B};
        return AC_OK;
    }
    {
        ProfScope ps(h, st, "lstm_step_kernel", 2.0 * T * (double)B * 4 * D * D * nroles,
                     (double)T * nroles * ((double)B * 4 * D * 4 + 4.0 * D * D * 4 + 2.0 * B * D * 4), nlaunch);
        for (int s = 0; s < nlaunch; ++s) {
            LstmLaunchParams q{};
            q.B = B;
            q.D = D;
            auto fill_last = [&](LstmRole& r, int t) {
                r.skip = x.p + (long long)t * x.ts;
                r.skip_bs = x.bs;
                r.yout = out.raw ? out.raw + (long long)t * D : nullptr;
                r.yout_elu = out.elu ? out.elu + (long long)t * D : nullptr;
                r.y_bs = (long long)T * D;
            };
            {
                LstmRole& r = q.role[0];
                r.active = s < T;
                r.kind = 0;
                r.a = s > 0 ? ws.hseq0 + (long long)(s - 1) * BD : nullptr;
                r.wpk = h->blob + lp.hh_off[0];
                r.gin = ws.gin + (long long)s * B4D;
                r.hnext = ws.hseq0 + (long long)s * BD;
                r.c = ws.c;
                r.first = s == 0;
                if (L == 1 && r.active) fill_last(r, s);
            }
            if (L == 2) {
                const int t1 = s - 1, t2 = s - 2;
                LstmRole& pr = q.role[1];
                pr.active = t1 >= 0 && t1 < T;
                pr.kind = 1;
                pr.a = ws.hseq0 + (long long)std::max(t1, 0) * BD;
                pr.wpk = h->blob + lp.ihpk_off[1];
                pr.bias = h->blob + lp.ih[1].b_off;
                pr.gout = ws.gin1 + (long long)std::max(t1, 0) * B4D;
                LstmRole& r = q.role[2];
                r.active = t2 >= 0 && t2 < T;
                r.kind = 0;
                r.a = t2 > 0 ? ws.hseq1 + (long long)(t2 - 1) * BD : nullptr;
                r.wpk = h->blob + lp.hh_off[1];
                r.gin = ws.gin1 + (long long)std::max(t2, 0) * B4D;
                r.hnext = ws.hseq1 + (long long)std::max(t2, 0) * BD;
                r.c = ws.c + (long long)B * D;
                r.first = t2 == 0;
                if (r.active) fill_last(r, t2);
            }
            const dim3 grid(D / 4, cdiv(B, 32), nroles), block(256);
            switch (D / 32) {
                case 2: hipLaunchKernelGGL(lstm_step_kernel<2>, grid, block, 0, st, q); break;
                case 4: hipLaunchKernelGGL(lstm_step_kernel<4>, grid, block, 0, st, q); break;
                case 8: hipLaunchKernelGGL(lstm_step_kernel<8>, grid, block, 0, st, q); break;
                default: hipLaunchKernelGGL(lstm_step_kernel<16>, grid, block, 0, st, q); break;
            }
        }
    }
    HIPCHK(h, hipGetLastError());
    const unsigned* am = amax_plus(h, st, x, 1.0f, B);
    y->raw = Act{out.raw, (long long)T * D, D, T, D, am, B};
    y->elu = Act{out.elu, (long long)T * D, D, T, D, am, B};
    return AC_OK;
}


int rvq_encode_fwd(ac_handle* h, hipStream_t st, const float* feats, int F, int K, long long* toks) {
    RvqEncParams p{};
    p.x = feats;
    p.epk = h->blob + h->cb_packed;
    p.e = h->blob + h->cb_plain;
    p.ee = h->blob + h->cb_ee;
    p.toks = toks;
    p.F = F;
    p.H = h->cfg.hidden_size;
    p.C = h->cfg.codebook_size;
    p.K = K;
    p.xs = p.H;
    p.tK = K;
    p.tk0 = 0;
    const int HV = p.H / 16;
    const int MS = (HV <= 8 && F >= 1024 * 32) ? 3 : 1;
    const dim3 grid(cdiv(F, 16 * MS)), block(64);
    const bool exact_env = h->dev.rvq_exact != 0;
// ... 113 lines not shown
    if (h->sticky) {
        volatile unsigned* s = h->sticky;
        const unsigned a = s[ST_LSTM_TIMEOUT], b = s[ST_LSTM_PLACEMENT], t = s[ST_BAD_TOKEN];
        if (a || b || t) {
            s[ST_LSTM_TIMEOUT] = 0;
            s[ST_LSTM_PLACEMENT] = 0;
            s[ST_BAD_TOKEN] = 0;
            char lstm[400] = "", tok[200] = "";
            if (a || b) {
                h->lstm_step_only = true;
                std::snprintf(lstm, sizeof lstm,
                              "an EARLIER call's persistent LSTM launch failed (%u bounded waits expired, %u launches without 32 workgroups on "
                              "every XCD -- is the GPU shared?): that call's outputs were set to NaN; the handle now uses the per-step LSTM "
                              "kernels, repeat the call", a, b);
            }
            if (t) std::snprintf(tok, sizeof tok, "an EARLIER ac_decode / ac_dequantize call got %u token ids outside [0, codebook_size): those frames were set to NaN", t);
            return fail(h, (a || b) ? AC_EHIP : AC_EINVAL, "%s%s%s", lstm, (a || b) && t ? "; ALSO: " : "", tok);
        }
    }
    return AC_OK;
}


int check_len(ac_handle* h, long long samples) {
    const long long lim = 0x70000000LL / (h->arch == ARCH_DAC ? 512 : 256) - 1;
    if (samples > lim) return fail(h, AC_EINVAL, "clip of %lld samples is too long for one call (limit %lld): split it", samples, lim);
    return AC_OK;
}


int encoder_fwd(ac_handle* h, hipStream_t st, const float* sig, const float* rel_len, int B, int T, float* feats, WsPtrs& ws) {
    const ac_config& c = h->cfg;
    const bool dbg = h->dbg != nullptr;
    Act xin{sig, (long long)T, 1, T, 1};
    Act2 x, y;
    int rc;
    auto rb_self_elu = [&](int C) {
        if (h->noncausal && h->gemm_fp32) return false;
        return (C == 32 || C == 64 || (C == 128 && c.num_ratios > 2 && rb128_ok(h, h->enc_rb[2]))) && c.residual_kernel_size == 3 && c.compress == 2;
    };
    auto rb256_self_elu = [&](int i, int L) { return i < c.num_ratios && h->enc_rb[i].C == h->enc_down[i - 1].N && rb256_ok(h, h->enc_rb[i], L); };
    int i0 = 0;
    if (enc_front_ok(h, T)) {
        float* d0 = dbg ? ws.take() : nullptr;
        float* d1 = dbg ? ws.take() : nullptr;
        rc = enc_front_fwd(h, st, sig, rel_len, B, T, ws.take(), d0, d1, &x);
        if (rc) return rc;
        if (dbg) {
            capture(h, st, Act{d0, (long long)T * 32, 32, T, 32}, B);
            capture(h, st, Act{d1, (long long)T * 32, 32, T, 32}, B);
            ws.give(d0);
            ws.give(d1);
        }
        capture(h, st, x.raw, B);
        i0 = 1;
    } else {
    if (thin_ok(c, c.kernel_size))
        rc = stem_fwd(h, st, sig, rel_len, B, T, Out{ws.take(), rb_self_elu(c.num_filters) ? nullptr : ws.take()}, &x);
    else
        rc = conv_fwd(h, st, h->enc_stem, xin, c.kernel_size, 1, rel_len, Out{ws.take(), ws.take()},
                      (long long)T * c.num_filters, c.num_filters, B, &x);
    if (rc) return rc;
    capture(h, st, x.raw, B);
    }
    for (int i = i0; i < c.num_ratios; ++i) {
        const int ratio = c.upsampling_ratios[c.num_ratios - 1 - i];
        float* hb = ws.take();
        rc = resblock_fwd(h, st, h->enc_rb[i], x, hb, Out{dbg ? ws.take() : nullptr, ws.take()}, B, &y);
        if (rc) return rc;
        ws.give(hb);
        ws.give(x);
        if (dbg) { capture(h, st, y.raw, B); ws.give(y.raw.p); y.raw.p = nullptr; }
        x = y;
        const int M = cdiv(x.elu.L, ratio);
        const bool last = i == c.num_ratios - 1;
        rc = conv_fwd(h, st, h->enc_down[i], x.elu, 2 * ratio, ratio, nullptr,
                      Out{ws.take(), (last || rb_self_elu(h->enc_down[i].N) || rb256_self_elu(i + 1, M)) ? nullptr : ws.take()},
                      (long long)M * h->enc_down[i].N, h->enc_down[i].N, B, &y);
        if (rc) return rc;
        ws.give(x);
        x = y;
        capture(h, st, x.raw, B);
    }
    rc = lstm_fwd(h, st, h->enc_lstm, x.raw, ws.lstm, Out{dbg ? ws.take() : nullptr, ws.take()}, B, &y);
    if (rc) return rc;
    ws.give(x);
    if (dbg) { capture(h, st, y.raw, B); ws.give(y.raw.p); y.raw.p = nullptr; }
    x = y;
    rc = conv_fwd(h, st, h->enc_final, x.elu, c.last_kernel_size, 1, nullptr, Out{feats, nullptr},
                  (long long)x.elu.L * c.hidden_size, c.hidden_size, B, nullptr);
    ws.give(x);
    return rc;
}


int decoder_fwd(ac_handle* h, hipStream_t st, const long long* toks, int B, int N, int K, float* sig, WsPtrs& ws) {
    const ac_config& c = h->cfg;
    const bool dbg = h->dbg != nullptr;
    float* zb = ws.take();
    int rc = rvq_decode_fwd(h, st, toks, B * N, K, zb);
    if (rc) return rc;
    Act z{zb, (long long)N * c.hidden_size, c.hidden_size, N, c.hidden_size};
    Act2 x, y;
    rc = conv_fwd(h, st, h->dec_first, z, c.kernel_size, 1, nullptr, Out{ws.take(), nullptr}, (long long)N * h->D, h->D, B, &x);
    if (rc) return rc;
    ws.give(zb);
    capture(h, st, x.raw, B);
    rc = lstm_fwd(h, st, h->dec_lstm, x.raw, ws.lstm, Out{dbg ? ws.take() : nullptr, ws.take()}, B, &y);
    if (rc) return rc;
    ws.give(x);
    if (dbg) { capture(h, st, y.raw, B); ws.give(y.raw.p); y.raw.p = nullptr; }
    x = y;
    for (int i = 0; i < c.num_ratios; ++i) {
        if (i == c.num_ratios - 1 && dec_tail_ok(h, x.elu)) {
            const long long T2 = 2LL * x.elu.L;
            float* d0 = dbg ? ws.take() : nullptr;
            float* d1 = dbg ? ws.take() : nullptr;
            rc = dec_tail_fwd(h, st, x.elu, B, sig, d0, d1);
            if (rc) return rc;
            if (dbg) {
                capture(h, st, Act{d0, T2 * 32, 32, (int)T2, 32}, B);
                capture(h, st, Act{d1, T2 * 32, 32, (int)T2, 32}, B);
                ws.give(d0);
                ws.give(d1);
            }
            ws.give(x);
            return AC_OK;
        }
        const int cup = h->dec_up[i].N / c.upsampling_ratios[i];
        const bool self_elu = ((cup == 32 || cup == 64 || (cup == 128 && rb128_ok(h, h->dec_rb[i]))) && c.residual_kernel_size == 3 &&
                               c.compress == 2) ||
                              (cup == h->dec_rb[i].C && rb256_ok(h, h->dec_rb[i], x.elu.L * c.upsampling_ratios[i]));
        rc = convtr_fwd(h, st, h->dec_up[i], x.elu, c.upsampling_ratios[i], Out{ws.take(), self_elu ? nullptr : ws.take()}, B, &y);
        if (rc) return rc;
        ws.give(x);
        x = y;
        capture(h, st, x.raw, B);
        float* hb = ws.take();
        rc = resblock_fwd(h, st, h->dec_rb[i], x, hb, Out{dbg ? ws.take() : nullptr, ws.take()}, B, &y);
        if (rc) return rc;
        ws.give(hb);
        ws.give(x);
        if (dbg) { capture(h, st, y.raw, B); ws.give(y.raw.p); y.raw.p = nullptr; }
        x = y;
    }
    if (thin_ok(c, c.last_kernel_size) && x.elu.ts == c.num_filters)
        rc = head_fwd(h, st, x.elu, B, sig);
    else
        rc = conv_fwd(h, st, h->dec_head, x.elu, c.last_kernel_size, 1, nullptr, Out{sig, nullptr}, (long long)x.elu.L, 1, B, nullptr);
    ws.give(x);
    return rc;
}

int mimi_linear(ac_handle* h, hipStream_t st, const PackedGemm& g, const float* x, long long rows, int cin, int x_pitch, int kofs,
                float* y, int y_pitch, const Epi& epi) {
    const long long widest = std::max<long long>(std::max(x_pitch, y_pitch), g.N);
    long long chunk = ((1LL << 31) / 4 - 4096) / widest / 128 * 128;
    if (chunk < 128) return fail(h, AC_EINVAL, "linear layer too wide for the tap-GEMM (%lld)", widest);
    for (long long r0 = 0; r0 < rows; r0 += chunk) {
        const long long n = std::min(chunk, rows - r0);
        TapGemmParams p{};
        p.nseg = 1;
        Act xa{x + r0 * x_pitch, 0, x_pitch, (int)n, cin};
        const bool one = r0 == 0 && n == rows;
        if (one && epi.rowmax_in) { xa.amax = epi.rowmax_in; xa.amax_n = -(int)n; }
        p.seg[0] = make_seg(xa, 1, 1, PAD_ZERO, 0, kofs, nullptr);
        if (one && epi.rowmax_out) p.amax_out_rows = reinterpret_cast<unsigned*>(1);
        p.amax_rows = 1;
        p.w = h->blob + g.w_off;
        p.bias = g.has_bias ? h->blob + g.b_off : nullptr;
        p.y = y + r0 * y_pitch;
        p.y_bs = 0;
        p.y_rs = y_pitch;
        p.B = 1;
        p.M = (int)n;
        p.N = g.N;
        p.Ktot = g.Ktot;
        p.scale = epi.scale;
        p.res = epi.res ? epi.res + r0 * epi.res_rs : nullptr;
        p.res_bs = 0;
        p.res_rs = epi.res_rs;
        p.gelu = epi.gelu;
        if (int rc = run_tap(h, st, p)) return rc;
        if (epi.rowmax_out) *epi.rowmax_out = one ? p.amax_out_rows : nullptr;
    }
    return AC_OK;
}

int upload_blob(ac_handle* h, Packer& pk, int device) {
    HIPCHK(h, hipSetDevice(device));
    hipDeviceProp_t prop;
// ... 126 lines not shown
```

### audiocodecs_amd/csrc/lstm_persist.h

```cpp
#pragma once
#include "lstm_consts.h"
#include <hip/hip_runtime.h>
#include "lstm.h"

namespace ac {


struct LstmPersistParams {
    const float* gin0;
    const float* w_pk;
    const float* bias1;
    float* hseq0;
    float* hseq1;
    const float* skip;
    float* yout;
    float* yout_elu;
    unsigned* ctl;
    long long gin_ts, h_ts, skip_bs, y_bs;
    int B, T;
    int group0;
    int clip0;
    int dbg;
};

constexpr int LP_CTL_SLOTS = 0;
constexpr int LP_CTL_TIMEOUT = 8 * 16;
constexpr int LP_CTL_FLAGS = 9 * 16;
constexpr int LP_CTL_WORDS = LP_CTL_FLAGS + 4 * 2 * LP_SLICES * LP_FLAG_STRIDE;

typedef unsigned u32x4_lp __attribute__((ext_vector_type(4)));
#define LP_RLX __ATOMIC_RELAXED, __HIP_MEMORY_SCOPE_AGENT
constexpr int LP_SC1 = 16;
constexpr int LP_SC0 = 1;

__device__ __forceinline__ unsigned lp_xcc_id() { return __builtin_amdgcn_s_getreg((3 << 11) | 20) & 0xf; }

__global__ __launch_bounds__(256) void lstm_persist_probe_kernel(unsigned* hist) {
    if (threadIdx.x == 0) atomicAdd(&hist[lp_xcc_id() & 15], 1u);
}

constexpr int LP_NEVER = 0x7f7f7f7f;

struct LstmTailParams {
    const unsigned* ctl;
    unsigned* sticky;
    const int* poison;
    float* yout;
    float* yout_elu;
    long long y_bs;
    int clip0, B, T, D;
    int xcds_used;
};

__global__ __launch_bounds__(256) void lstm_tail_kernel(const LstmTailParams p) {
    const int b = blockIdx.x;
    const unsigned tmo = p.ctl[LP_CTL_TIMEOUT];
    bool placed = true;
    for (int x = 0; x < 8; ++x) {
        const unsigned n = p.ctl[LP_CTL_SLOTS + x * 16];
        placed = placed && (x < p.xcds_used ? n == 32u : n <= 32u);
    }
    const bool failed = tmo != 0u || !placed;
    if (failed && b == 0 && blockIdx.y == 0 && threadIdx.x == 0)
        __hip_atomic_fetch_add(&p.sticky[(tmo == 2u || !placed) ? ST_LSTM_PLACEMENT : ST_LSTM_TIMEOUT], 1u, __ATOMIC_RELAXED, __HIP_MEMORY_SCOPE_SYSTEM);
    int t0 = p.T;
    if (failed) t0 = 0;
    else if (p.poison) {
        const int q = p.poison[p.clip0 + b];
        if (q < p.T) {
            t0 = q;
            if (blockIdx.y == 0 && threadIdx.x == 0)
                __hip_atomic_fetch_add(&p.sticky[ST_NONFINITE_CLIPS], 1u, __ATOMIC_RELAXED, __HIP_MEMORY_SCOPE_SYSTEM);
        }
    }
    if (t0 >= p.T) return;
    const float nan = __uint_as_float(0x7fc00000u);
    const long long n = (long long)(p.T - t0) * p.D;
    const long long o = (long long)(p.clip0 + b) * p.y_bs + (long long)t0 * p.D;
    for (long long i = (long long)blockIdx.y * 256 + threadIdx.x; i < n; i += 256LL * gridDim.y) {
        if (p.yout) p.yout[o + i] = nan;
        if (p.yout_elu) p.yout_elu[o + i] = nan;
    }
}

__device__ __forceinline__ bool lp_wait(unsigned* flags, unsigned want, unsigned* tmo, int lane, int dbg = 0) {
    if (AC_DEV_MODE(dbg, 4)) return true;
    for (unsigned spins = 0;; ++spins) {
        const unsigned f = lane < LP_SLICES ? __hip_atomic_load(&flags[lane * LP_FLAG_STRIDE], LP_RLX) : 0xffffffffu;
        if (__all(f >= want)) return true;
        if ((spins & 1023) == 1023 && __hip_atomic_load(tmo, LP_RLX)) return false;
        if (spins > (1u << 22)) { __hip_atomic_store(tmo, 1u, LP_RLX); return false; }
    }
}

__global__ __launch_bounds__(256) void lstm_persist_kernel(const LstmPersistParams p) {
    constexpr int D = LP_D;
    __shared__ float part[4][4][16][17];
    __shared__ unsigned s_x, s_slot;
    __shared__ int s_okp, s_okr;
    const int tid = threadIdx.x, lane = tid & 63, wave = tid >> 6;
    const int li = lane & 15, kq = lane >> 4;
    unsigned* tmo = p.ctl + LP_CTL_TIMEOUT;
    if (tid == 0) {
        s_x = lp_xcc_id();
        s_slot = __hip_atomic_fetch_add(&p.ctl[LP_CTL_SLOTS + (s_x & 7) * 16], 1u, LP_RLX);
    }
    __syncthreads();
    const int x = s_x & 7, slot = s_slot;
    const int g = x >> 1;
    const int G = (p.B + 15) >> 4;
    if (slot >= 32) {
        if (tid == 0) __hip_atomic_store(tmo, 2u, LP_RLX);
        return;
    }
    if (g >= G) return;
    if (AC_DEV_MODE(p.dbg, 1) && (slot >> 4) == 1) return;
    const int layer = slot >> 4, idx = (x & 1) * 16 + (slot & 15), u0 = idx * 16;

    f32x4 wa[4][8], wb[4][8];
    {
        const long long mat = (long long)LP_SLICES * 4 * 4 * 8 * 256;
        const float* base = p.w_pk + ((long long)idx * 4 + wave) * (4 * 8 * 256) + lane * 4;
        const float* pa = base + (layer == 0 ? 0 : mat);
        const float* pb = base + 2 * mat;
#pragma unroll
        for (int n = 0; n < 4; ++n)
#pragma unroll
            for (int ks = 0; ks < 8; ++ks) {
                wa[n][ks] = *reinterpret_cast<const f32x4*>(pa + (n * 8 + ks) * 256);
                wb[n][ks] = layer ? *reinterpret_cast<const f32x4*>(pb + (n * 8 + ks) * 256) : f32x4{0.f, 0.f, 0.f, 0.f};
            }
    }
    unsigned* flags0 = p.ctl + LP_CTL_FLAGS + ((g * 2 + 0) * LP_SLICES) * LP_FLAG_STRIDE;
    unsigned* flags1 = p.ctl + LP_CTL_FLAGS + ((g * 2 + 1) * LP_SLICES) * LP_FLAG_STRIDE;
    unsigned* myflag = (layer ? flags1 : flags0) + idx * LP_FLAG_STRIDE;
    float* hmine = layer ? p.hseq1 : p.hseq0;
    const long long goff = (long long)(p.group0 + g) * (D / 16) * 256;

    const int ec = tid >> 4, ej = tid & 15;
    const int eb = g * 16 + ec;
    const bool live = eb < p.B;
    const long long erow = (long long)(p.clip0 + eb);
    const int eu = u0 + ej;
    float cstate = 0.f;
    float bq[4] = {0.f, 0.f, 0.f, 0.f};
    if (layer == 1) {
#pragma unroll
        for (int q = 0; q < 4; ++q) bq[q] = p.bias1[q * D + eu];
    }
    const int hpos = (((ej >> 2) << 4) + ec) * 4 + (ej & 3);

    auto load_a = [&](const float* seq, int t, f32x4 (&a)[8]) {
        const float* src = seq + (long long)t * p.h_ts + goff + (long long)(wave * 8) * 256;
        const __amdgpu_buffer_rsrc_t rs = __builtin_amdgcn_make_buffer_rsrc((void*)src, 0, 8 * 1024, 0x00020000);
#pragma unroll
        for (int ks = 0; ks < 8; ++ks) a[ks] = __builtin_bit_cast(f32x4, __builtin_amdgcn_raw_buffer_load_b128(rs, (ks * 64 + lane) * 16, 0, LP_SC1));
    };
    f32x4 accP[4];
    auto project = [&](int t) -> bool {
        if (wave == 0) { const bool ok = lp_wait(flags0, (unsigned)(t + 1), tmo, lane, p.dbg); if (lane == 0) s_okp = ok; }
        __syncthreads();
        if (!s_okp) return false;
        f32x4 a[8];
        load_a(p.hseq0, t, a);
// ... 86 lines not shown
```

### audiocodecs_amd/csrc/lstm_persist16.h

```cpp
#pragma once
#include "lstm_persist.h"
#include "tap_gemm6.h"
#include "rb_fused6.h"
#include <type_traits>

namespace ac {

constexpr int LP16_SLICE_BYTES = 2 * 16 * 16 * 2;
constexpr long long LP16_GROUP_BYTES = (long long)LP_SLICES * LP16_SLICE_BYTES;
#ifndef LP16_RING_N
#define LP16_RING_N 8
#endif
constexpr int LP16_RING = LP16_RING_N;
static_assert(LP16_RING >= 4 && (LP16_RING & (LP16_RING - 1)) == 0, "ring of the recurrent exchange: a power of two, >= 4 (see above)");

struct LstmPersist16Params {
    LstmPersistParams base;
    const __bf16* w_pk6;
    const float* bias0;
    int fuse_in;
    int* poison;
    const float* winv;
    const unsigned* amax_x;
    void* hseq0_local;
// ... 145 lines not shown
    };
    auto load_valid = [&](const char* seq, int t, bf16x8 (&a)[2][2]) -> bool {
        for (unsigned spins = 0;; ++spins) {
            load_a(seq, t, a);
            if (valid(a) || AC_DEV_MODE(p.dbg, 4)) return true;
            if ((spins & 63) == 63 && __hip_atomic_load(tmo, LP_RLX)) return false;
            if (spins > (1u << 18)) { __hip_atomic_store(tmo, 1u, LP_RLX); return false; }
            __builtin_amdgcn_s_sleep(4);
        }
    };
    bf16x8 arec[2][2];
    float skip_next = 0.f;
    f32x4 accP[4];
    const bool xlive = g * 16 + li < p.B;
    const __amdgpu_buffer_rsrc_t xrs = __builtin_amdgcn_make_buffer_rsrc(
        (void*)(p.skip + (long long)(p.clip0 + g * 16) * p.skip_bs), 0, (int)(((long long)(p.B - g * 16 < 16 ? p.B - g * 16 : 16)) * p.skip_bs * 4), 0x00020000);
    const int xoff = xlive ? (int)((long long)li * p.skip_bs * 4) + (wave * 64 + 8 * kq) * 4 : 0x7fff0000;
    f32x4 xr[2][2];
    auto fetch0 = [&](int t) {
#pragma unroll
        for (int ks = 0; ks < 2; ++ks)
#pragma unroll
            for (int hf = 0; hf < 2; ++hf)
                xr[ks][hf] = bufload16(xrs, xlive ? xoff + (t * D + ks * 32 + hf * 4) * 4 : 0x7fff0000, 0);
    };
    float xsc = 1.f, xcr[4] = {1.f, 1.f, 1.f, 1.f};
    if (fuse0) {
        const int cb = p.clip0 + g * 16, cl = p.clip0 + p.B - 1;
        xsc = s16_pow2(s16_exponent(*amax_at(pp.amax_x, cb + li <= cl ? cb + li : cl)));
#pragma unroll
        for (int r = 0; r < 4; ++r) xcr[r] = s16_pow2(LP16_HEXP - s16_exponent(*amax_at(pp.amax_x, cb + kq * 4 + r <= cl ? cb + kq * 4 + r : cl)));
    }
    bf16x8 xa[2][2];
    auto convert0 = [&]() {
        bf16x8 (&a)[2][2] = xa;
#pragma unroll
        for (int ks = 0; ks < 2; ++ks) {
            typedef _Float16 f16x4v __attribute__((ext_vector_type(4)));
            const f32x4 s0 = xr[ks][0] * xsc, s1 = xr[ks][1] * xsc;
            const f16x4v h0 = __builtin_convertvector(s0, f16x4v), h1 = __builtin_convertvector(s1, f16x4v);
            const f16x4v l0 = __builtin_convertvector(s0 - __builtin_convertvector(h0, f32x4), f16x4v);
            const f16x4v l1 = __builtin_convertvector(s1 - __builtin_convertvector(h1, f32x4), f16x4v);
            a[ks][0] = __builtin_bit_cast(bf16x8, __builtin_shufflevector(h0, h1, 0, 1, 2, 3, 4, 5, 6, 7));
            a[ks][1] = __builtin_bit_cast(bf16x8, __builtin_shufflevector(l0, l1, 0, 1, 2, 3, 4, 5, 6, 7));
        }
    };
    auto project0 = [&](int t, int trec, auto rec_tag) {
        bf16x8 (&a)[2][2] = xa;
#pragma unroll
        for (int n = 0; n < 4; ++n) accP[n] = f32x4{0.f, 0.f, 0.f, 0.f};
        if constexpr (decltype(rec_tag)::value && !LATE) load_a(hmine, rt(trec), arec);
        mac(a, wb, accP, 0, 1);
        mac(a, wb, accP, 1, 2);
#pragma unroll
        for (int n = 0; n < 4; ++n)
#pragma unroll
            for (int r = 0; r < 4; ++r) accP[n][r] *= xcr[r];
        if constexpr (decltype(rec_tag)::value && LATE) {
            __builtin_amdgcn_sched_barrier(0);
            await_publish(trec);
            load_a(hmine, rt(trec), arec);
        }
        (void)t;
    };
    auto project = [&](int t) -> bool {
        bf16x8 a[2][2];
        if (!load_valid(h0b, t, a)) return false;
#pragma unroll
        for (int n = 0; n < 4; ++n) accP[n] = f32x4{0.f, 0.f, 0.f, 0.f};
        mac(a, wa, accP);
        return true;
    };
#pragma unroll
    for (int n = 0; n < 4; ++n) accP[n] = f32x4{0.f, 0.f, 0.f, 0.f};
    if (layer == 1 && !project(0)) return;
    if (fuse0) {
        fetch0(0);
        convert0();
        project0(0, 0, std::false_type{});
        fetch0(p.T > 1 ? 1 : 0);
    }
    const float* skip_row = p.skip + (live ? erow : (long long)p.clip0) * p.skip_bs + eu;
    if (layer == 1) skip_next = skip_row[0];
    bf16x8 ap[2][2];
    if (layer == 1) load_a(h0b, p.T > 1 ? 1 : 0, ap);

    const bool trc = AC_DEV_MODE(p.dbg, 32) && idx == 0 && tid == 0;
    unsigned long long* trw = reinterpret_cast<unsigned long long*>(p.ctl + LP_CTL_FLAGS) + (g * 2 + layer) * 64;
#define LP16_TRC(pt_) do { if (trc && t >= 100 && t < 104) trw[(t - 100) * 8 + (pt_)] = __builtin_amdgcn_s_memrealtime(); } while (0)
    auto step = [&](int t) -> bool {
        if (trc && t >= 100 && t < 104) { trw[(t - 100) * 8 + 6] = 0; trw[(t - 100) * 8 + 7] = 0; }
        LP16_TRC(0);
        if (trc && (t == 100 || t == 103)) trw[32 + (t == 103)] = __builtin_amdgcn_s_memtime();
        float gpre[4] = {bq[0], bq[1], bq[2], bq[3]};
        const float skipv = skip_next;
        if (live && layer == 0 && !FUSE) {
            const float* gp = p.gin0 + (long long)t * p.gin_ts + erow * (4 * D);
#pragma unroll
            for (int q = 0; q < 4; ++q) gpre[q] = gp[q * D + eu];
        }
        f32x4 acc[4];
#pragma unroll
        for (int n = 0; n < 4; ++n) acc[n] = accP[n];
        if (t > 0) {
            const bool first_ok = (layer == 1 || fuse0) && (valid(arec) || AC_DEV_MODE(p.dbg, 4));
            if (trc && !first_ok) trw[63] += 1;
            if (!first_ok && !load_valid(hmine, rt(t - 1), arec)) return false;
            LP16_TRC(1);
            if (layer == 0) mac(arec, wa, acc);
            else mac(arec, wb, acc);
        }
        bool ap_ok = true;
        if (fuse0) {
            convert0();
            fetch0(t + 2 < p.T ? t + 2 : p.T - 1);
        }
        if (layer == 1) ap_ok = valid(ap) || AC_DEV_MODE(p.dbg, 4);
        LP16_TRC(2);
        f32x4 (&pt)[8][16][LP16_PART_PITCH] = part[t & 1];
#pragma unroll
        for (int r = 0; r < 4; ++r) pt[wave][kq * 4 + r][li] = f32x4{acc[0][r], acc[1][r], acc[2][r], acc[3][r]};
        lds_barrier();
        LP16_TRC(3);
        float hn = 0.f;
        if (gate_thr) {
            float pre[4];
            f32x4 pv[8];
#pragma unroll
            for (int w = 0; w < 8; ++w) pv[w] = pt[w][ec][ej];
#pragma unroll
            for (int q = 0; q < 4; ++q) {
                const float sum = ((pv[0][q] + pv[1][q]) + (pv[2][q] + pv[3][q])) + ((pv[4][q] + pv[5][q]) + (pv[6][q] + pv[7][q]));
                pre[q] = __fmaf_rn(sum, wiv[q], gpre[q]);
            }
            const float ig = sigmoid_rcp(pre[0]), fg = sigmoid_rcp(pre[1]), gg = tanh_rcp(pre[2]), og = sigmoid_rcp(pre[3]);
            cstate = fg * cstate + ig * gg;
            hn = og * tanh_rcp(cstate);
            LP16_TRC(6);
            const bool nonfinite = !(fabsf(hn) < 2.0f);
            if (nonfinite && live) atomicMin(pp.poison + erow, t);
            const float hp = nonfinite ? 0.f : hn;
            const float h2 = LP16_HSCALE * hp;
            _Float16 hh = (_Float16)h2;
            if (LP16_HEXP && fabsf((float)hh) >= 2.0f) hh = (_Float16)copysignf(1.9990234375f, h2);
            const _Float16 hl = (_Float16)(h2 - (float)hh);
            char* dst = hmine + (long long)rt(t) * p.h_ts + goff + (long long)idx * SLICE_BYTES;
            const __amdgpu_buffer_rsrc_t rs = __builtin_amdgcn_make_buffer_rsrc((void*)dst, 0, SLICE_BYTES, 0x00020000);
            __builtin_amdgcn_raw_buffer_store_b16(__builtin_bit_cast(unsigned short, hh), rs, hpos, 0, LP_SC0);
            __builtin_amdgcn_raw_buffer_store_b16(__builtin_bit_cast(unsigned short, hl), rs, 512 + hpos, 0, LP_SC0);
            LP16_TRC(7);
            if (lane == 0) pubflag[wave] = (unsigned)t + 1u;
            if (t >= 2) {
                char* old = hmine + (long long)rt(t - 2) * p.h_ts + goff + (long long)idx * SLICE_BYTES;
                const __amdgpu_buffer_rsrc_t ro = __builtin_amdgcn_make_buffer_rsrc((void*)old, 0, SLICE_BYTES, 0x00020000);
                __builtin_amdgcn_raw_buffer_store_b16((unsigned short)0xFFFFu, ro, hpos, 0, LP_SC0);
                __builtin_amdgcn_raw_buffer_store_b16((unsigned short)0xFFFFu, ro, 512 + hpos, 0, LP_SC0);
            }
            if (layer == 0) {
                hist[t % LP16_BATCH][0][tid] = __builtin_bit_cast(unsigned short, hh);
                hist[t % LP16_BATCH][1][tid] = __builtin_bit_cast(unsigned short, hl);
            }
        }
        LP16_TRC(4);
        if (layer == 0 && gate_thr && ((t + 1) % LP16_BATCH == 0 || t + 1 == p.T)) {
            for (int tb = t - (t % LP16_BATCH); tb <= t; ++tb) {
                const __amdgpu_buffer_rsrc_t rx = __builtin_amdgcn_make_buffer_rsrc((void*)(h0b + (long long)tb * p.h_ts + goff + (long long)idx * SLICE_BYTES), 0, SLICE_BYTES, 0x00020000);
#pragma unroll
                for (int pl = 0; pl < NP; ++pl) __builtin_amdgcn_raw_buffer_store_b16(hist[tb % LP16_BATCH][pl][tid], rx, pl * 512 + hpos, 0, LP_SC1);
            }
        }
        if (layer == 1) {
            if (live) {
                const float yv = hn + skipv;
                const long long o = erow * p.y_bs + (long long)t * D + eu;
                if (p.yout) p.yout[o] = yv;
                if (p.yout_elu) p.yout_elu[o] = elu1(yv);
            }
            const int t1 = t + 1 < p.T ? t + 1 : t;
            if (!ap_ok && !load_valid(h0b, t1, ap)) return false;
#pragma unroll
            for (int n = 0; n < 4; ++n) accP[n] = f32x4{0.f, 0.f, 0.f, 0.f};
            if constexpr (!LATE) load_a(hmine, rt(t), arec);
            mac(ap, wa, accP, 0, 1);
            if constexpr (!LATE) skip_next = skip_row[(long long)t1 * D];
            mac(ap, wa, accP, 1, 2);
            if constexpr (LATE) {
                __builtin_amdgcn_sched_barrier(0);
                await_publish(t);
                load_a(hmine, rt(t), arec);
                skip_next = skip_row[(long long)t1 * D];
            }
            load_a(h0b, t + 2 < p.T ? t + 2 : t1, ap);
        } else if (fuse0) {
            project0(t + 1 < p.T ? t + 1 : t, t, std::true_type{});
        }
        LP16_TRC(5);
        return true;
    };
    for (int t = 0; t < p.T; ++t)
        if (!step(t)) return;
#undef LP16_TRC
    };
    if (wave < 4) {
        if (layer_rt == 0) body(std::integral_constant<int, 0>{}, std::false_type{});
        else body(std::integral_constant<int, 1>{}, std::false_type{});
    } else {
        if (layer_rt == 0) body(std::integral_constant<int, 0>{}, std::true_type{});
        else body(std::integral_constant<int, 1>{}, std::true_type{});
    }
}

}
```

### audiocodecs_amd/csrc/tap_gemm.h

```cpp
#pragma once
#include <hip/hip_runtime.h>
#include <stdint.h>

namespace ac {

typedef float f32x4 __attribute__((ext_vector_type(4)));

struct TapSeg {
    const float* x;
    long long bs;
    long long ts;
    const float* rel_len;
    int L;
    int cin;
    int cin_shift;
    int s;
    int J;
    int Lp;
    int lim;
    int reflect;
    int elu;
    int kofs;
    int pad;
    int dil;
    const unsigned* amax;
    int amax_n;
};

struct TapGemmParams {
    TapSeg seg[2];
    int nseg;
    const float* w;
    const float* bias;
    float* y;
    float* y_elu;
    long long y_bs, y_rs;
    int B, M, N, Ktot;
    int mtiles, ntiles;
    const float* scale;
    const float* res;
    long long res_bs, res_rs;
    int gelu;
    const float* alpha;
    const float* alpha_inv;
    int alpha_n;
    int tanh_out;
    long long y_off, y_len;
    int n_valid;
    const float* winv;
    unsigned* amax_out;
    int amax_rows;
    unsigned* amax_out_rows;
    int epi_direct;
    int stagger;
    unsigned long long* clk;
};

enum { PAD_ZERO = 0, PAD_REFLECT = 1, PAD_REPLICATE = 2 };

__device__ __forceinline__ float gelu1(float v) {
    const float u = v * 0.70710678118654752440f;
    const float t = fabsf(u);
    float p = 4.536090636975132e-05f;
    p = fmaf(p, t, -0.00044552396866492927f);
    p = fmaf(p, t, 0.001489486894570291f);
    p = fmaf(p, t, 0.0007745670736767352f);
    p = fmaf(p, t, -0.02825363539159298f);
    p = fmaf(p, t, 0.1484815925359726f);
    p = fmaf(p, t, 0.9184163808822632f);
    p = fmaf(p, t, 1.6279085874557495f);
    const float er = copysignf(1.0f - __builtin_amdgcn_exp2f(-(p * t)), u);
    const float hv = 0.5f * v;
    return fmaf(hv, er, hv);
}

__device__ __forceinline__ float elu1(float v) { return v > 0.f ? v : (__expf(v) - 1.0f); }

__device__ __forceinline__ f32x4 elu4(f32x4 v) {
    v.x = elu1(v.x); v.y = elu1(v.y); v.z = elu1(v.z); v.w = elu1(v.w);
    return v;
}

__device__ __forceinline__ float sin2_f32(float t) {
    if (__builtin_expect(!(__builtin_fabsf(t) < 32768.f), 0)) {
        const float s = sinf(t);
        return __fmul_rn(s, s);
    }
    const float k = __builtin_rintf(__fmul_rn(t, 0.636619747f));
    float r = __fmaf_rn(k, -0x1.921fb6p+0f, t);
    r = __fmaf_rn(k, 0x1.777a5cp-25f, r);
    r = __fmaf_rn(k, 0x1.ee59dap-50f, r);
    const float z = __fmul_rn(r, r);
    float q = __fmaf_rn(2.7181215500604594e-06f, z, -0.00019839312881231308f);
    q = __fmaf_rn(q, z, 0.008333329111337662f);
    q = __fmaf_rn(q, z, -0.1666666716337204f);
    const float sn = __fmaf_rn(__fmul_rn(r, z), q, r);
    const float s2 = __fmul_rn(sn, sn);
    return ((int)k & 1) ? __fsub_rn(1.f, s2) : s2;
}
__device__ __forceinline__ float snake1(float v, float a, float ainv) {
    return __fadd_rn(v, __fmul_rn(ainv, sin2_f32(__fmul_rn(a, v))));
}

__device__ __forceinline__ float act1(const TapGemmParams& p, float v, int n) {
    if (p.alpha) {
        const int c = n % p.alpha_n;
        return snake1(v, p.alpha[c], p.alpha_inv[c]);
    }
    return elu1(v);
}

__device__ __forceinline__ float epilogue1(const TapGemmParams& p, float v, int n, long long res_off) {
    if (p.gelu) v = gelu1(v);
    if (p.scale) v = __fmul_rn(p.scale[n], v);
    if (p.res) v = __fadd_rn(p.res[res_off], v);
    if (p.tanh_out) v = tanhf(v);
    return v;
}

constexpr int GEN_EXTRA = 56;
constexpr int KC = 32;
constexpr int KCP = KC + 4;
constexpr int T6_DIL_HALO = 56;

__device__ __forceinline__ long long src_index(const TapSeg& sg, int i) {
    if (i >= sg.lim) return -1;
    int j = i;
    if (sg.reflect == PAD_REFLECT) {
        if (j < 0) j = -j;
        else if (j >= sg.Lp) j = 2 * (sg.Lp - 1) - j;
    } else if (sg.reflect == PAD_REPLICATE) {
        j = j < 0 ? 0 : (j >= sg.L ? sg.L - 1 : j);
    }
    if (j < 0 || j >= sg.L) return -1;
    return j;
}
// ... 136 lines not shown
```

### audiocodecs_amd/csrc/tap_gemm8.h

```cpp
#pragma once
#include "tap_gemm6.h"

namespace ac {

template <int WGM, int WGN, int WMT, int WN>
struct Tap8Cfg {
    using C6 = Tap6Cfg<WGM, WGN, WMT, WN, 7>;
    static_assert(WGM * WGN == 8, "8 waves");
    static constexpr int BM = C6::BM, BN = C6::BN, NT = C6::NT, A_ROWS = C6::A_ROWS, A_SLOTS = C6::A_SLOTS, PLANE = C6::PLANE;
    static constexpr int NTILES = BN / 32;
    static constexpr int B_PIECES = 2 * NTILES * 2;
    static constexpr int B_SLOT = B_PIECES * 512;
    static constexpr int PPW = B_PIECES / 8;
    static_assert(B_PIECES % 8 == 0, "fragments divide over the 8 waves");
    static constexpr size_t a_bytes = (size_t)2 * 2 * PLANE * 2;
    static constexpr size_t b_bytes = (size_t)2 * B_SLOT * 2;
    static_assert(a_bytes % 16 == 0, "ring base alignment");
    static constexpr size_t main_bytes = a_bytes + b_bytes;
    static constexpr size_t lds_bytes = main_bytes > C6::epi_bytes ? main_bytes : C6::epi_bytes;
    static_assert(lds_bytes <= 160 * 1024, "one workgroup per CU: slabs + weight ring (or the staged epilogue's tile) within 160 KB of LDS");
};

__device__ __forceinline__ void t8_glds16(const void* gsrc, unsigned lds_dst) {
#ifdef T8_ABL_NODMA
    return;
#endif
    unsigned keep;
    asm volatile("s_mov_b32 %0, m0\n\ts_mov_b32 m0, %2\n\ts_nop 0\n\tglobal_load_lds_dwordx4 %1, off\n\ts_mov_b32 m0, %0"
                 : "=&s"(keep) : "v"(gsrc), "s"(lds_dst) : "memory");
}
template <int N>
__device__ __forceinline__ void t8_wait() {
    asm volatile("s_waitcnt vmcnt(%0)" ::"n"(N) : "memory");
}

template <int WGM, int WGN, int WMT, int WN, bool RM, bool J1, bool SPREAD = true>
__global__ __launch_bounds__(512, 1) void tap_gemm8_kernel(const TapGemmParams p, const __bf16* __restrict__ wp) {
    using Cfg = Tap8Cfg<WGM, WGN, WMT, WN>;
    constexpr int BM = Cfg::BM, BN = Cfg::BN, NT = Cfg::NT, A_SLOTS = Cfg::A_SLOTS, PLANE = Cfg::PLANE, NTILES = Cfg::NTILES;
    constexpr int HALO = 7;
    unsigned long long clk_t0 = 0, clk_r0 = 0;
    if (p.clk) { clk_t0 = __builtin_amdgcn_s_memtime(); clk_r0 = __builtin_amdgcn_s_memrealtime(); }
    extern __shared__ __attribute__((aligned(16))) float smem[];
    __bf16* As0 = reinterpret_cast<__bf16*>(smem);
    __bf16* Bs0 = reinterpret_cast<__bf16*>(reinterpret_cast<char*>(smem) + Cfg::a_bytes);
    const unsigned bs_lds = (unsigned)(size_t)Bs0;

    const int tid = threadIdx.x, lane = tid & 63;
    const int wave = __builtin_amdgcn_readfirstlane(tid >> 6);
    const int wm = wave / WGN, wn = wave % WGN;
    const int i32 = lane & 31, kh = lane >> 5;

    int id;
    {
        const int total = gridDim.x, q = total >> 3, r = total & 7, xcd = blockIdx.x & 7, pos = blockIdx.x >> 3;
        id = (xcd < r ? xcd * (q + 1) : r * (q + 1) + (xcd - r) * q) + pos;
    }
    const int nt = id % p.ntiles; id /= p.ntiles;
    const int mt = id % p.mtiles;
    const int b = id / p.mtiles;
    const int m0 = mt * BM, n0 = nt * BN;
#ifdef T6_TRACE
    const bool t6_ph = p.clk && mt == p.mtiles / 2 && nt == 0 && b == p.B / 2 && tid == 64;
    const bool t8_on = p.clk && mt == p.mtiles / 2 && nt == 0 && b == p.B / 2 && lane == 0;
    int t8_stage = 0;
    if (t6_ph) p.clk[4] = clk_t0;
#define T8_STAMP(k) do { if (t8_on && t8_stage < 16) p.clk[16 + (wave * 16 + t8_stage) * 8 + (k)] = __builtin_amdgcn_s_memtime(); } while (0)
#define T8_USTAMP(u) do { if (t8_on && (t8_stage == 2 || t8_stage == 3) && (u) < 8) p.clk[16 + (wave * 16 + 8 + (u)) * 8 + 3 + t8_stage] = __builtin_amdgcn_s_memtime(); } while (0)
    T6_PHASE(1);
#else
    const bool t6_ph = false;
#define T8_STAMP(k) do { } while (0)
#define T8_USTAMP(u) do { } while (0)
#endif

    const TapSeg& sg = p.seg[0];
    const unsigned am_early = RM ? 0u : *amax_at(sg.amax, b);
    const int seg_J = sg.J, seg_Cw = sg.s * sg.cin, seg_kofs = sg.kofs, rowstep = sg.dil;
    const int NC = seg_Cw / KC;
    const long long lo_t = (long long)m0 * sg.s - sg.pad;
    const long long hi_t = (long long)(m0 + BM - 1 + (sg.J - 1) * sg.dil) * sg.s + (sg.s - 1) - sg.pad;
    const bool inside = lo_t >= 0 && hi_t < sg.L;
    const bool seg_interior = inside || sg.s == 1;
    const int tsf = sg.s == 1 ? (int)sg.ts : sg.cin;
    const __amdgpu_buffer_rsrc_t a_rs = __builtin_amdgcn_make_buffer_rsrc((void*)(sg.x + (long long)b * sg.bs), 0,
                                                                             (int)(((long long)(sg.L - 1) * sg.ts + sg.cin) * 4), 0x00020000);
    const int R = BM + (sg.J - 1) * sg.dil;
    int a_boff[A_SLOTS];
    const int a_lds0 = (tid / (KC / 4)) * T6_PITCH + 4 * (tid % (KC / 4));
    const bool last_slot_ok = (tid + (A_SLOTS - 1) * NT) / (KC / 4) < Cfg::A_ROWS;
    unsigned a_zero = 0;
#pragma unroll
    for (int i = 0; i < A_SLOTS; ++i) {
        const int e = tid + i * NT;
        const int row = e / (KC / 4), q = e % (KC / 4);
        long long t = (long long)(m0 + (row < R ? row : 0)) * sg.s - sg.pad;
        if (!inside) {
            if (sg.s == 1) {
                const long long jj = row < R ? src_index(sg, (int)t) : 0;
                if (jj < 0) a_zero |= 1u << i;
                t = jj < 0 ? 0 : jj;
            } else {
                t = 0;
            }
        }
        a_boff[i] = (int)((t * tsf + 4 * q) * 4);
    }
    __builtin_amdgcn_sched_barrier(0);
    float a_scale = 1.f, a_inv = 1.f;
    float a_rsc[RM ? A_SLOTS : 1];
    constexpr bool rowmode = RM;
    if (!RM) {
        unsigned am = am_early;
        asm volatile("" : "+v"(am));
        const int se = s16_exponent(am);
        a_scale = s16_pow2(se);
        a_inv = s16_pow2(-se);
        a_rsc[0] = a_scale;
    } else {
#pragma unroll
        for (int i = 0; i < A_SLOTS; ++i) {
            const int m = m0 + (tid + i * NT) / (KC / 4);
            a_rsc[RM ? i : 0] = s16_pow2(s16_exponent(sg.amax[m < p.M ? m : p.M - 1]));
        }
    }

    f32x16 acc[WMT][WN];
#pragma unroll
// ... 1 lines not shown
#pragma unroll
        for (int c = 0; c < WN; ++c)
#pragma unroll
            for (int r = 0; r < 16; ++r) acc[a][c][r] = 0.f;

    constexpr int A_OOB = 0x7fff0000;
    const __amdgpu_buffer_rsrc_t a_rs_null = __builtin_amdgcn_make_buffer_rsrc((void*)(sg.x + (long long)b * sg.bs), 0, 0, 0x00020000);
    auto load_a = [&](int c, bool live, f32x4 (&ra)[A_SLOTS]) {
#ifdef T8_ABL_NOALOAD
        live = false;
#endif
        const int c_ = c * KC;
        if (seg_interior || !live) {
            const int soff = __builtin_amdgcn_readfirstlane(live ? c_ * 4 : 0);
            const __amdgpu_buffer_rsrc_t rs = live ? a_rs : a_rs_null;
#pragma unroll
            for (int i = 0; i < A_SLOTS; ++i) ra[i] = bufload16(rs, a_boff[i], soff);
        } else {
            int voff[A_SLOTS];
#pragma unroll
            for (int i = 0; i < A_SLOTS; ++i) {
                const int e = tid + i * NT;
                const int row = e / (KC / 4), q = e % (KC / 4);
                const int cc = c_ + 4 * q;
                const int tp = sg.cin_shift >= 0 ? (cc >> sg.cin_shift) : (cc / sg.cin);
                const long long jj = row < R ? src_index(sg, (m0 + row) * sg.s + tp - sg.pad) : -1;
                voff[i] = jj < 0 ? A_OOB : (int)((jj * sg.ts + (cc - tp * sg.cin)) * 4);
            }
#pragma unroll
            for (int i = 0; i < A_SLOTS; ++i) ra[i] = bufload16(a_rs, voff[i], 0);
        }
    };
    auto load_slot = [&](int c, bool live, f32x4 (&ra)[A_SLOTS], int i) {
#ifdef T8_ABL_NOALOAD
        live = false;
#endif
        const int c_ = c * KC;
        if (seg_interior || !live) {
            const int soff = __builtin_amdgcn_readfirstlane(live ? c_ * 4 : 0);
            const __amdgpu_buffer_rsrc_t rs = live ? a_rs : a_rs_null;
            ra[i] = bufload16(rs, a_boff[i], soff);
        } else {
            const int e = tid + i * NT;
            const int row = e / (KC / 4), q = e % (KC / 4);
            const int cc = c_ + 4 * q;
            const int tp = sg.cin_shift >= 0 ? (cc >> sg.cin_shift) : (cc / sg.cin);
            const long long jj = row < R ? src_index(sg, (m0 + row) * sg.s + tp - sg.pad) : -1;
            ra[i] = bufload16(a_rs, jj < 0 ? A_OOB : (int)((jj * sg.ts + (cc - tp * sg.cin)) * 4), 0);
        }
    };
    auto store_slot = [&](const f32x4 (&ra)[A_SLOTS], __bf16* dst, int i) {
        if (i + 1 == A_SLOTS) asm volatile("" ::"v"(ra[i]));
#ifdef T8_ABL_NOSTORE
        return;
#endif
        if (i + 1 < A_SLOTS || last_slot_ok) {
            const f32x4 v = (a_zero & (1u << i)) ? f32x4{0.f, 0.f, 0.f, 0.f} : ra[i];
            split16_store4s(v, a_rsc[RM ? i : 0], dst, PLANE, a_lds0 + i * (NT / (KC / 4)) * T6_PITCH);
        }
    };
    auto store_a = [&](const f32x4 (&ra)[A_SLOTS], __bf16* dst) {
#pragma unroll
        for (int i = 0; i < A_SLOTS; ++i) store_slot(ra, dst, i);
    };
    const int ksteps = p.Ktot >> 4;
    const __bf16* wtile = wp + (long long)(n0 >> 5) * ksteps * 1024 + lane * 8;
    auto issue_b = [&](int c, int j, int slot) {
        const int k0 = (seg_kofs + j * seg_Cw + c * KC) >> 4;
#pragma unroll
        for (int i = 0; i < Cfg::PPW; ++i) {
            const int f = wave * Cfg::PPW + i;
            const int ks = f / (2 * NTILES), t = (f / 2) % NTILES, pl = f % 2;
            t8_glds16(wtile + ((long long)t * ksteps + k0 + ks) * 1024 + pl * 512, bs_lds + (unsigned)((slot * Cfg::B_PIECES + f) * 1024));
        }
    };

    auto issue_piece = [&](int c, int j, int slot, int i) {
        const int k0 = (seg_kofs + j * seg_Cw + c * KC) >> 4;
        const int f = wave * Cfg::PPW + i;
        const int ks = f / (2 * NTILES), t = (f / 2) % NTILES, pl = f % 2;
        t8_glds16(wtile + ((long long)t * ksteps + k0 + ks) * 1024 + pl * 512, bs_lds + (unsigned)((slot * Cfg::B_PIECES + f) * 1024));
    };

    const int a_frag = (wm * WMT * 32 + i32) * T6_PITCH + 8 * kh;
    auto compute = [&](int abuf, int jr, int slot, auto&& hook) {
        const __bf16* Ac = As0 + abuf * 2 * PLANE + a_frag + jr * T6_PITCH;
        const __bf16* Bc = Bs0 + slot * Cfg::B_SLOT + lane * 8;
        f16x8 bf[2][2][WN], af[2][2];
        auto read_b = [&](int ks, f16x8 (&dst)[2][WN]) {
#pragma unroll
            for (int c = 0; c < WN; ++c)
#pragma unroll
                for (int pl = 0; pl < 2; ++pl) dst[pl][c] = *reinterpret_cast<const f16x8*>(Bc + ((ks * NTILES + wn * WN + c) * 2 + pl) * 512);
        };
        auto read_a = [&](int ks, int a, f16x8 (&dst)[2]) {
#pragma unroll
            for (int pl = 0; pl < 2; ++pl) dst[pl] = *reinterpret_cast<const f16x8*>(Ac + pl * PLANE + a * 32 * T6_PITCH + ks * 16);
        };
        read_b(0, bf[0]);
        read_a(0, 0, af[0]);
#pragma unroll
        for (int u = 0; u < 2 * WMT; ++u) {
            const int ks = u / WMT, a = u % WMT;
            if (u + 1 < 2 * WMT) read_a((u + 1) / WMT, (u + 1) % WMT, af[(u + 1) & 1]);
            if (a == WMT - 1 && ks == 0) read_b(1, bf[1]);
#pragma unroll
            for (int c = 0; c < WN; ++c) {
#ifdef T8_ABL_NOMFMA
                asm volatile("" ::"v"(af[u & 1][0]), "v"(af[u & 1][1]), "v"(bf[ks][0][c]), "v"(bf[ks][1][c]));
#else
                f32x16 v = acc[a][c];
                v = __builtin_amdgcn_mfma_f32_32x32x16_f16(af[u & 1][1], bf[ks][0][c], v, 0, 0, 0);
                v = __builtin_amdgcn_mfma_f32_32x32x16_f16(af[u & 1][0], bf[ks][1][c], v, 0, 0, 0);
                acc[a][c] = __builtin_amdgcn_mfma_f32_32x32x16_f16(af[u & 1][0], bf[ks][0][c], v, 0, 0, 0);
#endif
            }
            hook(u);
            __builtin_amdgcn_sched_barrier(0);
            T8_USTAMP(u);
        }
    };
    auto no_hook = [](int) {};
    constexpr int UNITS = 2 * WMT;
    constexpr int SPU = (A_SLOTS + UNITS - 1) / UNITS, SU0 = UNITS - (A_SLOTS + SPU - 1) / SPU;
    auto store_hook = [&](const f32x4 (&ra)[A_SLOTS], __bf16* dst, bool st, int u) {
        if (u >= SU0 && st) {
#pragma unroll
            for (int k = 0; k < SPU; ++k)
                if ((u - SU0) * SPU + k < A_SLOTS) store_slot(ra, dst, (u - SU0) * SPU + k);
        }
    };

    auto tasks = [&](int u, bool has_next, int nc, int nj, int nslot, bool issue, int creq, f32x4 (&ra_req)[A_SLOTS], bool store, const f32x4 (&ra_st)[A_SLOTS], __bf16* dst,
                     auto issue_tag, auto store_tag) {
        constexpr bool ISSUE = decltype(issue_tag)::value, STORE = decltype(store_tag)::value;
        constexpr int NTASK = Cfg::PPW + (ISSUE ? A_SLOTS : 0) + (STORE ? A_SLOTS : 0);
        const int lo = u * NTASK / UNITS, hi = (u + 1) * NTASK / UNITS;
#pragma unroll
        for (int t = 0; t < NTASK; ++t) {
            if (t < lo || t >= hi) continue;
            if (t < Cfg::PPW) {
                if (has_next) issue_piece(nc, nj, nslot, t);
            } else if (ISSUE && t < Cfg::PPW + A_SLOTS) {
                load_slot(creq, issue, ra_req, t - Cfg::PPW);
            } else {
                if (store) store_slot(ra_st, dst, t - Cfg::PPW - (ISSUE ? A_SLOTS : 0));
            }
        }
    };

    using T = std::true_type;
    using F = std::false_type;
#pragma unroll
    for (int i = 0; i < (RM ? A_SLOTS : 1); ++i) asm volatile("" ::"v"(a_rsc[i]));
#ifdef T6_TRACE
    T6_PHASE(2);
#endif
    if constexpr (J1) {
        f32x4 raA[A_SLOTS], raB[A_SLOTS];
        issue_b(0, 0, 0);
        load_a(0, true, raA);
        load_a(1, NC > 1, raB);
        store_a(raA, As0);
        t8_wait<A_SLOTS>();
        lds_barrier();
#ifdef T6_TRACE
        T6_PHASE(6);
#endif
        auto stage = [&](int c, f32x4 (&ra_next)[A_SLOTS], f32x4 (&ra_free)[A_SLOTS]) {
            T8_STAMP(0);
            const bool st = c + 1 < NC;
            __bf16* dst = As0 + ((c + 1) & 1) * 2 * PLANE;
            if constexpr (SPREAD) {
                T8_STAMP(1);
                compute(c & 1, 0, c & 1, [&](int u) { tasks(u, c + 1 < NC, c + 1, 0, (c + 1) & 1, c + 2 < NC, c + 2, ra_free, st, ra_next, dst, T{}, T{}); });
            } else {
                if (c + 1 < NC) issue_b(c + 1, 0, (c + 1) & 1);
                load_a(c + 2, c + 2 < NC, ra_free);
                __builtin_amdgcn_sched_barrier(0);
                T8_STAMP(1);
                compute(c & 1, 0, c & 1, [&](int u) { store_hook(ra_next, dst, st, u); });
            }
            __builtin_amdgcn_sched_barrier(0);
            T8_STAMP(2);
            t8_wait<A_SLOTS>();
            T8_STAMP(3);
            lds_barrier();
            T8_STAMP(4);
#ifdef T6_TRACE
            ++t8_stage;
#endif
        };
        for (int c = 0; c < NC; c += 2) {
            stage(c, raB, raA);
            if (c + 1 < NC) stage(c + 1, raA, raB);
        }
    } else {
        f32x4 ra[A_SLOTS];
        issue_b(0, 0, 0);
        load_a(0, true, ra);
        store_a(ra, As0);
        load_a(1, NC > 1, ra);
        t8_wait<A_SLOTS>();
        lds_barrier();
#ifdef T6_TRACE
        T6_PHASE(6);
#endif
        auto stage = [&](int c, int j, auto store_tag, auto issue_tag) {
            constexpr bool STORE = decltype(store_tag)::value, ISSUE = decltype(issue_tag)::value;
            const int s = c * seg_J + j;
            int nc = c, nj = j + 1;
            if (nj == seg_J) { nj = 0; nc = c + 1; }
            T8_STAMP(0);
            if constexpr (SPREAD) {
                T8_STAMP(1);
                const bool st = c + 1 < NC;
                __bf16* dst = As0 + ((c + 1) & 1) * 2 * PLANE;
                compute(c & 1, j * rowstep, s & 1, [&](int u) { tasks(u, nc < NC, nc, nj, (s + 1) & 1, c + 2 < NC, c + 2, ra, st, ra, dst, issue_tag, store_tag); });
            } else {
            if (nc < NC) issue_b(nc, nj, (s + 1) & 1);
            if (ISSUE) load_a(c + 2, c + 2 < NC, ra);
            __builtin_amdgcn_sched_barrier(0);
            T8_STAMP(1);
            if constexpr (STORE) {
                const bool st = c + 1 < NC;
                __bf16* dst = As0 + ((c + 1) & 1) * 2 * PLANE;
                compute(c & 1, j * rowstep, s & 1, [&](int u) { store_hook(ra, dst, st, u); });
            } else {
                compute(c & 1, j * rowstep, s & 1, no_hook);
            }
            }
            __builtin_amdgcn_sched_barrier(0);
            T8_STAMP(2);
            if (ISSUE) t8_wait<A_SLOTS>(); else t8_wait<0>();
            T8_STAMP(3);
            lds_barrier();
            T8_STAMP(4);
#ifdef T6_TRACE
            ++t8_stage;
#endif
        };
// ... 14 lines not shown
```

### audiocodecs_amd/csrc/tap_route.h

```cpp
#pragma once
#include "core.h"

namespace acimpl {

struct TapRouteInputs {
    bool w6 = false;
    bool winv = false;
    bool want_rowmode = false;
    bool want_rows = false;
    bool gemm_fp32 = false;
};

enum class TapFamily { scalar, vec, tap4, tap6, tap6_dil, tap8 };

enum { TK_RM = 1, TK_J1 = 2, TK_SPREAD = 4 };
constexpr int tap_key(int wgm, int wgn, int wm, int wn, int flags = 0) { return flags << 16 | wgm << 12 | wgn << 8 | wm << 4 | wn; }

struct TapRoute {
    int reject_taps = 0;
    TapFamily family = TapFamily::scalar;
    int wgm = 0, wgn = 0, wm = 0, wn = 0;
    int form8 = 0;
    bool rm = false, j1 = false, spread = false;
    bool rowmode = false;
    bool rows_out = false;
    bool epi_direct = false;
    bool dil_slab = false;
    char name[48] = "";
    int key() const { return tap_key(wgm, wgn, wm, wn, (rm ? TK_RM : 0) | (j1 ? TK_J1 : 0) | (spread ? TK_SPREAD : 0)); }
};

inline void tap_route_set(TapRoute& r, TapFamily f, int wgm, int wgn, int wm, int wn) {
    r.family = f;
    r.wgm = wgm;
    r.wgn = wgn;
    r.wm = wm;
    r.wn = wn;
    const char* fmt = f == TapFamily::scalar   ? "tap_gemm_kernel<%d, %d, %d, %d, false>"
                      : f == TapFamily::vec    ? "tap_gemm_kernel<%d, %d, %d, %d, true>"
                      : f == TapFamily::tap4   ? "tap_gemm4_kernel<%d, %d, %d, %d>"
                      : f == TapFamily::tap6   ? "tap_gemm6_kernel<%d, %d, %d, %d, 2>"
                      : f == TapFamily::tap6_dil ? "tap_gemm6_kernel<%d, %d, %d, %d, 2, dil>"
                                                 : "tap_gemm8_kernel<%d, %d, %d, %d, 2>";
    std::snprintf(r.name, sizeof r.name, fmt, wgm, wgn, wm, wn);
}

inline TapRoute route_tap(const TapGemmParams& p, const TapRouteInputs& in, const ac_handle::DevSwitches& dev) {
    TapRoute r;
    bool vec = (p.Ktot % 4 == 0) && aligned16(p.w);
    bool fast = vec && (p.N % 4 == 0) && (p.y_rs % 4 == 0) && (p.y_bs % 4 == 0) && (!p.y || aligned16(p.y)) &&
                (!p.y_elu || aligned16(p.y_elu)) && (long long)p.N * p.Ktot * 4 < (1LL << 31);
    for (int i = 0; i < p.nseg; ++i) {
        const TapSeg& s = p.seg[i];
        vec = vec && (s.cin % 4 == 0) && (s.ts % 4 == 0) && (s.bs % 4 == 0) && (s.kofs % 4 == 0) && aligned16(s.x);
        fast = fast && ((s.s * s.cin) % KC == 0) && (s.ts == s.cin || s.s == 1) && !s.rel_len && !s.elu &&
               ((long long)(s.L - 1) * s.ts + s.cin) * 4 < (1LL << 31);
        if (s.J > 8) {
            r.reject_taps = s.J;
            return r;
        }
    }
    fast = fast && vec;
    double kk = 0;
    for (int i = 0; i < p.nseg; ++i) kk += (double)p.seg[i].J * p.seg[i].s * p.seg[i].cin;
    bool use6 = fast && !in.gemm_fp32 && (p.N % 64 == 0 || p.N % 96 == 0) && in.w6;
    for (int i = 0; use6 && i < p.nseg; ++i) use6 = p.seg[i].kofs % 32 == 0;
    if (!use6) {
        const TapFamily f = fast ? TapFamily::tap4 : vec ? TapFamily::vec : TapFamily::scalar;
        if (p.N <= 16) tap_route_set(r, f, 4, 1, 2, 1);
        else if (p.N <= 32) tap_route_set(r, f, 4, 1, 2, 2);
        else if (p.N <= 64) tap_route_set(r, f, 2, 2, 2, 2);
        else if (p.N % 96 == 0 && p.N % 128 != 0) tap_route_set(r, f, 2, 2, 4, 3);
        else tap_route_set(r, f, 2, 2, 4, 4);
        return r;
    }
    r.rowmode = in.want_rowmode && in.winv && p.B == 1 && p.nseg == 1 && p.seg[0].J == 1 && p.seg[0].s == 1 && p.seg[0].pad == 0 &&
                p.seg[0].lim >= p.M && p.seg[0].L >= p.M && p.y_off == 0;
    r.rows_out = r.rowmode && in.want_rows;
    if (!r.rowmode && in.winv) {
        const bool staged_env = dev.tap_epi_staged != 0;
        r.epi_direct = !staged_env && !p.gelu && !p.scale && !p.tanh_out && p.y_off == 0 && p.y_len == 0 &&
                       (!p.res || (p.alpha && (long long)p.M * p.res_rs * 4 < 0x7fffffffLL && p.res_rs * 4 < (1 << 20))) && (!p.alpha || p.y_elu) &&
                       (p.n_valid == 0 || p.n_valid == p.N) && (p.alpha ? p.N < 128 && p.N % 32 == 0 : p.N % 128 == 0) &&
                       (long long)p.M * p.y_rs * 4 < 0x7fffffffLL && p.y_rs * 4 < (1 << 20);
    }
    const bool dil_env = dev.tap_dil != 0;
    r.dil_slab = dil_env && !r.rowmode && p.nseg == 1 && p.seg[0].dil != 1    && p.seg[0].s == 1 && (p.seg[0].J - 1) * p.seg[0].dil <= T6_DIL_HALO;
    const TapSeg& s0 = p.seg[0];
    const bool can8 = in.winv && p.nseg == 1 && (s0.J - 1) * s0.dil <= 7 && !(s0.dil != 1 && s0.s != 1) && p.N % 128 == 0 && (s0.s * s0.cin) % 32 == 0 &&
                      (!r.epi_direct || p.N % 128 == 0);
    const int want8 = dev.tap8;
    if (can8 && want8 != 0) {
        auto fill8 = [&](int bm, int bn) {
            const double w = (double)p.B * cdiv(p.M, bm) * (p.N / bn) / 256.0;
            return w / std::ceil(w) * ((double)p.M / ((double)cdiv(p.M, bm) * bm));
        };
        const double sc1 = p.N % 256 == 0 ? 1.00 * fill8(256, 256) : 0.0;
        const double sc3 = p.N % 256 == 0 ? 0.90 * fill8(128, 256) : 0.0;
        int form = sc1 >= sc3 ? 1 : 3;
        bool model = (form == 1 ? sc1 : sc3) >= 0.80;
        if (p.N % 256 != 0) {
            form = 2;
            model = kk >= 3072 && fill8(256, 128) >= 0.70;
        }
        if ((double)p.B * cdiv(p.M, 128) * (p.N / 128) <= 64.0) {
            form = p.N % 256 == 0 ? 3 : 2;
            model = true;
        }
        if (dev.tap8_form >= 1 && dev.tap8_form <= 3 && (dev.tap8_form == 2 || p.N % 256 == 0)) form = dev.tap8_form;
        if (want8 >= 1 || model) {
            r.form8 = form;
            if (form == 1) tap_route_set(r, TapFamily::tap8, 2, 4, 4, 2);
            else if (form == 3) tap_route_set(r, TapFamily::tap8, 2, 4, 2, 2);
            else tap_route_set(r, TapFamily::tap8, 4, 2, 2, 2);
            r.j1 = s0.J == 1;
            r.rm = r.j1 && r.rowmode;
            r.spread = dev.tap8_spread == 2 || (dev.tap8_spread == 1 && r.wgm * r.wm * 32 == 128);
            return r;
        }
    }
    int pick = 0;
    if (p.N % 256 == 0) {
        const double wg256 = (double)p.B * cdiv(p.M, 128) * (p.N / 256);
        auto fill = [](double wgs, double slots) { const double w = wgs / slots; return w / std::ceil(w); };
        const double s128 = in.winv ? 1.06 * fill(2.0 * wg256, 768.0) : 1.00 * fill(2.0 * wg256, 512.0);
        const double s256 = 1.10 * fill(wg256, 512.0);
        const double s8 = (kk >= 2048 ? (in.winv ? 1.00 : 1.12) : (in.winv ? 0.85 : 0.95)) * fill(wg256, 256.0);
        pick = s256 >= s128 && s256 >= s8 ? 1 : (s8 > s128 ? 2 : 0);
        if (dev.tap_pick >= 0 && dev.tap_pick <= 2) pick = dev.tap_pick;
    }
    auto tap6 = [&](int wgm, int wgn, int wmt, int wn) {
        const bool dil = in.winv && r.dil_slab && (wn >= 2 || (wgm == 1 && wgn == 4 && kk >= 2048));
        tap_route_set(r, dil ? TapFamily::tap6_dil : TapFamily::tap6, wgm, wgn, wmt, wn);
    };
    if (pick == 1) tap6(1, 4, 4, 2);
    else if (pick == 2) tap6(1, 8, 4, 1);
    else if (p.N % 128 == 0) tap6(1, 4, 4, 1);
    else if (p.N % 192 == 0) tap6(2, 2, 2, 3);
    else if (p.N % 96 == 0) tap6(4, 1, 1, 3);
    else tap6(2, 2, 2, 1);
    return r;
}

}
```

Baseline: 42290.

## Emit LSTM output as split16 planes consumed directly by tap8 conv kernel

The LSTM persist kernel can now write its ELU output pre-split into two fp16 planes. A new planes-input variant of tap_gemm8_kernel then streams these planes straight into LDS with async loads, using a zero row for padding. This skips the separate split/convert of the activation in the conv that follows the LSTM, in both encoder and decoder. It adds new kernel instantiations, a routing check, and an error path for routes that cannot take plane input.

```diff
diff --git a/audiocodecs_amd/csrc/ac_api.hip b/audiocodecs_amd/csrc/ac_api.hip
--- a/audiocodecs_amd/csrc/ac_api.hip
+++ b/audiocodecs_amd/csrc/ac_api.hip
@@ -65,6 +65,7 @@
     h->dev.tap8 = num("AC_TAP8", -1);
     h->dev.tap8_form = num("AC_TAP8_FORM", 0);
     h->dev.tap8_spread = num("AC_TAP8_SPREAD", 1);
+    h->dev.tap8_planes = num("AC_TAP8_PLANES", 1);
 #ifdef AC_DEVELOPER
     h->dev.rb6_dbg = num("AC_RB6_DBG", 0);
     h->dev.lstm_dbg = num("AC_LSTM_DBG", 0);
@@ -90,7 +91,7 @@
 int ac_debug_set(ac_handle* h, const char* key, int value) {
     if (!h || !key) return AC_EINVAL;
     struct { const char* k; int* v; } tab[] = {
-        {"tap_epi_staged", &h->dev.tap_epi_staged}, {"tap_dil", &h->dev.tap_dil}, {"tap_stagger", &h->dev.tap_stagger}, {"tap_pick", &h->dev.tap_pick}, {"tap8", &h->dev.tap8}, {"tap8_form", &h->dev.tap8_form}, {"tap8_spread", &h->dev.tap8_spread},
+        {"tap_epi_staged", &h->dev.tap_epi_staged}, {"tap_dil", &h->dev.tap_dil}, {"tap_stagger", &h->dev.tap_stagger}, {"tap_pick", &h->dev.tap_pick}, {"tap8", &h->dev.tap8}, {"tap8_form", &h->dev.tap8_form}, {"tap8_spread", &h->dev.tap8_spread}, {"tap8_planes", &h->dev.tap8_planes},
         {"rb6_dbg", &h->dev.rb6_dbg}, {"rb_stream", &h->dev.rb_stream}, {"chain_stream", &h->dev.chain_stream}, {"rb128_stream", &h->dev.rb128_stream}, {"rb256_fused", &h->dev.rb256_fused}, {"front_seg", &h->dev.front_seg}, {"tail_seg", &h->dev.tail_seg}, {"front_ldspad", &h->dev.front_ldspad},
         {"lstm_dbg", &h->dev.lstm_dbg}, {"lstm_fuse_in", &h->dev.lstm_fuse_in}, {"rvq_exact", &h->dev.rvq_exact}, {"prof_detail", &h->dev.prof_detail}, {"head_seq", &h->dev.head_seq}, {"attn_exact", &h->dev.attn_exact}, {"dac_unit", &h->dev.dac_unit}, {"mimi_tail", &h->dev.mimi_tail},
         {"mstream_skinny", &h->dev.mstream_skinny},
diff --git a/audiocodecs_amd/csrc/core.h b/audiocodecs_amd/csrc/core.h
--- a/audiocodecs_amd/csrc/core.h
+++ b/audiocodecs_amd/csrc/core.h
@@ -49,6 +49,8 @@
     bool has6 = false;
     bool hb256 = false;
 };
+
+constexpr int TAP8_ZROW_FLOATS = 1024;
 
 struct LstmPlan {
     int D, layers;
@@ -169,6 +171,7 @@
         int tap_pick = -1;
         int tap8 = -1;
         int tap8_form = 0;
+        int tap8_planes = 1;
         int tap8_spread = 1;
         int rb6_dbg = 0;
         int rb_stream = 1;
@@ -197,6 +200,7 @@
     bool noncausal = false;
     bool has_enc = true, has_dec = true;
     bool gemm_fp32 = false;
+    size_t zrow_off = 0;
     std::map<size_t, size_t> winv_of;
     std::map<const void*, int> mimi_streams;
     std::map<const void*, int> mimi_dstreams;
@@ -708,6 +712,7 @@
                 const size_t mat16 = (size_t)LP_SLICES * 4 * 4 * 4 * 2 * 512;
                 lp.persist16_off = reserve((4 * mat16 + 1) / 2);
                 lp.persist16_inv = reserve((size_t)2 * 4 * D);
+                if (!h->zrow_off) h->zrow_off = reserve(TAP8_ZROW_FLOATS);
                 std::vector<int> sc((size_t)2 * 4 * D);
                 const int layer_of[4] = {0, 1, 1, 0};
                 for (int l = 0; l < 2; ++l)
@@ -753,6 +758,7 @@
     int L, C;
     const unsigned* amax = nullptr;
     int amax_n = 0;
+    const float* zrow = nullptr;
 };
 
 int prof_name(ac_handle* h, const char* nm);
@@ -826,6 +832,9 @@
 
 int convtr_fwd(ac_handle* h, hipStream_t st, const PackedGemm& g, const Act& x, int s, Out out, int B, Act2* y);
 
+bool conv_planes_ok(const ac_handle* h, const PackedGemm& g, const Act& x, int k, int s, const float* rel_len, Out out, long long out_bs, long long out_rs, int B);
+bool convtr_planes_ok(const ac_handle* h, const PackedGemm& g, const Act& x, int s, Out out, int B);
+
 bool rb128_ok(const ac_handle* h, const ResBlockPlan& rb);
 
 int resblock_fwd(ac_handle* h, hipStream_t st, const ResBlockPlan& rb, const Act2& x, float* hbuf, Out out, int B, Act2* y);
@@ -858,7 +867,7 @@
     float *gin, *gin1, *hseq0, *hseq1, *c;
 };
 
-int lstm_fwd(ac_handle* h, hipStream_t st, const LstmPlan& lp, const Act& x, const LstmWs& ws, Out out, int B, Act2* y);
+int lstm_fwd(ac_handle* h, hipStream_t st, const LstmPlan& lp, const Act& x, const LstmWs& ws, Out out, int B, Act2* y, bool planes_out = false);
 
 int rvq_encode_fwd(ac_handle* h, hipStream_t st, const float* feats, int F, int K, long long* toks);
 
diff --git a/audiocodecs_amd/csrc/core.hip b/audiocodecs_amd/csrc/core.hip
--- a/audiocodecs_amd/csrc/core.hip
+++ b/audiocodecs_amd/csrc/core.hip
@@ -232,21 +232,28 @@
     return fail(h, AC_EINVAL, "run_tap: no instantiation of %s", r.name);
 }
 
-template <int WGM, int WGN, int WMT, int WN, bool RM, bool J1, bool SP>
+template <int WGM, int WGN, int WMT, int WN, bool RM, bool J1, bool SP, bool PL = false>
 static int launch_tap8(ac_handle* h, hipStream_t st, TapGemmParams& p, const __bf16* w6, const char* name, double flops, double bytes) {
     using Cfg = Tap8Cfg<WGM, WGN, WMT, WN>;
+    constexpr size_t lds = PL ? Cfg::pl_lds_bytes : Cfg::lds_bytes;
     p.mtiles = cdiv(p.M, Cfg::BM);
     p.ntiles = p.N / Cfg::BN;
     const long long blocks = (long long)p.B * p.mtiles * p.ntiles;
     ProfScope ps(h, st, name, flops, bytes);
-    if (int rc = ensure_lds(h, reinterpret_cast<const void*>(tap_gemm8_kernel<WGM, WGN, WMT, WN, RM, J1, SP>), Cfg::lds_bytes)) return rc;
-    hipLaunchKernelGGL((tap_gemm8_kernel<WGM, WGN, WMT, WN, RM, J1, SP>), dim3((unsigned)blocks), dim3(Cfg::NT), Cfg::lds_bytes, st, p, w6);
+    if (int rc = ensure_lds(h, reinterpret_cast<const void*>(tap_gemm8_kernel<WGM, WGN, WMT, WN, RM, J1, SP, PL>), lds)) return rc;
+    hipLaunchKernelGGL((tap_gemm8_kernel<WGM, WGN, WMT, WN, RM, J1, SP, PL>), dim3((unsigned)blocks), dim3(Cfg::NT), lds, st, p, w6);
     return AC_OK;
 }
 
 static int launch_tap8_family(ac_handle* h, hipStream_t st, TapGemmParams& p, const TapRoute& r, const __bf16* w6, const char* name, double flops, double bytes) {
-    constexpr int RJ = TK_RM | TK_J1, J = TK_J1, S = TK_SPREAD;
+    constexpr int RJ = TK_RM | TK_J1, J = TK_J1, S = TK_SPREAD, P = TK_PL;
     switch (r.key()) {
+    case tap_key(2, 4, 4, 2, P): return launch_tap8<2, 4, 4, 2, false, false, false, true>(h, st, p, w6, name, flops, bytes);
+    case tap_key(2, 4, 4, 2, P | S): return launch_tap8<2, 4, 4, 2, false, false, true, true>(h, st, p, w6, name, flops, bytes);
+    case tap_key(2, 4, 2, 2, P): return launch_tap8<2, 4, 2, 2, false, false, false, true>(h, st, p, w6, name, flops, bytes);
+    case tap_key(2, 4, 2, 2, P | S): return launch_tap8<2, 4, 2, 2, false, false, true, true>(h, st, p, w6, name, flops, bytes);
+    case tap_key(4, 2, 2, 2, P): return launch_tap8<4, 2, 2, 2, false, false, false, true>(h, st, p, w6, name, flops, bytes);
+    case tap_key(4, 2, 2, 2, P | S): return launch_tap8<4, 2, 2, 2, false, false, true, true>(h, st, p, w6, name, flops, bytes);
     case tap_key(2, 4, 4, 2, RJ): return launch_tap8<2, 4, 4, 2, true, true, false>(h, st, p, w6, name, flops, bytes);
     case tap_key(2, 4, 4, 2, RJ | S): return launch_tap8<2, 4, 4, 2, true, true, true>(h, st, p, w6, name, flops, bytes);
     case tap_key(2, 4, 4, 2, J): return launch_tap8<2, 4, 4, 2, false, true, false>(h, st, p, w6, name, flops, bytes);
@@ -298,17 +305,24 @@
 }
 
 
+static TapRouteInputs route_inputs(const ac_handle* h, const TapGemmParams& p) {
+    TapRouteInputs in;
+    in.w6 = h->w6_of.count((size_t)(p.w - h->blob)) != 0;
+    in.winv = h->winv_of.count((size_t)(p.w - h->blob)) != 0;
+    in.want_rowmode = p.amax_rows != 0;
+    in.want_rows = p.amax_out_rows != nullptr;
+    in.gemm_fp32 = h->gemm_fp32;
+    return in;
+}
+
 int run_tap(ac_handle* h, hipStream_t st, TapGemmParams& p) {
     const auto w6_it = h->w6_of.find((size_t)(p.w - h->blob));
     const auto iv = h->winv_of.find((size_t)(p.w - h->blob));
-    TapRouteInputs in;
-    in.w6 = w6_it != h->w6_of.end();
-    in.winv = iv != h->winv_of.end();
-    in.want_rowmode = p.amax_rows != 0;
-    in.want_rows = p.amax_out_rows != nullptr;
-    in.gemm_fp32 = h->gemm_fp32;
+    const TapRouteInputs in = route_inputs(h, p);
     const TapRoute r = route_tap(p, in, h->dev);
     if (r.reject_taps) return fail(h, AC_EINVAL, "conv with %d taps exceeds the kernel limit of 8", r.reject_taps);
+    if (r.reject_planes || (p.a_zrow && p.seg[0].amax_n != p.B))
+        return fail(h, AC_ESTATE, "run_tap: the activation operand holds split16 planes and %s does not take them", r.name);
     double kk = 0, inb = 0;
     for (int i = 0; i < p.nseg; ++i) {
         kk += (double)p.seg[i].J * p.seg[i].s * p.seg[i].cin;
@@ -405,11 +419,72 @@
 }
 
 
+static TapGemmParams conv_params(const ac_handle* h, const PackedGemm& g, const Act& x, int k, int s, const float* rel_len, Out out,
+                                 long long out_bs, long long out_rs, int B) {
+    const int M = cdiv(x.L, s);
+    const int extra = M * s - x.L;
+    TapGemmParams p{};
+    p.nseg = 1;
+    if (h->noncausal) {
+        const int total = k - s, right = total / 2;
+        p.seg[0] = make_seg(x, s, s == 1 ? k : 2, PAD_REFLECT, extra, 0, rel_len, total - right, right);
+    } else {
+        p.seg[0] = make_seg(x, s, s == 1 ? k : 2, PAD_REFLECT, extra, 0, rel_len);
+    }
+    p.a_zrow = x.zrow;
+    p.w = h->blob + g.w_off;
+    p.bias = g.has_bias ? h->blob + g.b_off : nullptr;
+    p.y = out.raw;
+    p.y_elu = out.elu;
+    p.y_bs = out_bs;
+    p.y_rs = out_rs;
+    p.B = B;
+    p.M = M;
+    p.N = g.N;
+    p.Ktot = g.Ktot;
+    return p;
+}
+
+static TapGemmParams convtr_params(const ac_handle* h, const PackedGemm& g, const Act& x, Out out, int B) {
+    TapGemmParams p{};
+    p.nseg = 1;
+    p.seg[0] = make_seg(x, 1, 2, PAD_ZERO, 0, 0, nullptr);
+    p.a_zrow = x.zrow;
+    p.w = h->blob + g.w_off;
+    p.bias = h->blob + g.b_off;
+    p.y = out.raw;
+    p.y_elu = out.elu;
+    p.y_bs = (long long)x.L * g.N;
+    p.y_rs = g.N;
+    p.B = B;
+    p.M = x.L;
+    p.N = g.N;
+    p.Ktot = g.Ktot;
+    return p;
+}
+
+static bool planes_route_ok(const ac_handle* h, TapGemmParams p, int B) {
+    if (!h->dev.tap8_planes || h->gemm_fp32 || !h->zrow_off || p.seg[0].cin > TAP8_ZROW_FLOATS) return false;
+    p.a_zrow = h->blob + h->zrow_off;
+    p.seg[0].amax = reinterpret_cast<const unsigned*>(h->blob);
+    p.seg[0].amax_n = B;
+    const TapRoute r = route_tap(p, route_inputs(h, p), h->dev);
+    return r.planes && !r.reject_planes;
+}
+bool conv_planes_ok(const ac_handle* h, const PackedGemm& g, const Act& x, int k, int s, const float* rel_len, Out out, long long out_bs, long long out_rs, int B) {
+    if (s != 1) return false;
+    return planes_route_ok(h, conv_params(h, g, x, k, s, rel_len, out, out_bs, out_rs, B), B);
+}
+bool convtr_planes_ok(const ac_handle* h, const PackedGemm& g, const Act& x, int s, Out out, int B) {
+    if (s == 2) return false;
+    return planes_route_ok(h, convtr_params(h, g, x, out, B), B);
+}
+
 int conv_fwd(ac_handle* h, hipStream_t st, const PackedGemm& g, const Act& x, int k, int s, const float* rel_len, Out out,
              long long out_bs, long long out_rs, int B, Act2* y) {
     const int M = cdiv(x.L, s);
     const int extra = M * s - x.L;
-    if (s == 2 && k == 4 && !rel_len && extra == 0 && x.L >= 4 && out_rs == 64 && out_bs == (long long)M * 64 && !h->noncausal) {
+    if (!x.zrow && s == 2 && k == 4 && !rel_len && extra == 0 && x.L >= 4 && out_rs == 64 && out_bs == (long long)M * 64 && !h->noncausal) {
         const unsigned* am = nullptr;
         const int rc = try_thin6(h, st, g, x, 32, 1, out, B, &am);
         if (rc <= 0) {
@@ -421,25 +496,8 @@
             return rc;
         }
     }
-    TapGemmParams p{};
-    p.nseg = 1;
     if (s != 1 && k != 2 * s) return fail(h, AC_EINVAL, "strided conv needs kernel == 2*stride (got k=%d, s=%d)", k, s);
-    if (h->noncausal) {
-        const int total = k - s, right = total / 2;
-        p.seg[0] = make_seg(x, s, s == 1 ? k : 2, PAD_REFLECT, extra, 0, rel_len, total - right, right);
-    } else {
-        p.seg[0] = make_seg(x, s, s == 1 ? k : 2, PAD_REFLECT, extra, 0, rel_len);
-    }
-    p.w = h->blob + g.w_off;
-    p.bias = g.has_bias ? h->blob + g.b_off : nullptr;
-    p.y = out.raw;
-    p.y_elu = out.elu;
-    p.y_bs = out_bs;
-    p.y_rs = out_rs;
-    p.B = B;
-    p.M = M;
-    p.N = g.N;
-    p.Ktot = g.Ktot;
+    TapGemmParams p = conv_params(h, g, x, k, s, rel_len, out, out_bs, out_rs, B);
     const int rc = run_tap(h, st, p);
     if (y) {
         y->raw = Act{out.raw, out_bs, out_rs, M, g.N, p.amax_out, p.B};
@@ -451,7 +509,7 @@
 
 int convtr_fwd(ac_handle* h, hipStream_t st, const PackedGemm& g, const Act& x, int s, Out out, int B, Act2* y) {
     const int cout = g.N / s;
-    if (s == 2) {
+    if (s == 2 && !x.zrow) {
         const unsigned* am = nullptr;
         const int rc = try_thin6(h, st, g, x, 64, 0, out, B, &am);
         if (rc <= 0) {
@@ -463,19 +521,7 @@
             return rc;
         }
     }
-    TapGemmParams p{};
-    p.nseg = 1;
-    p.seg[0] = make_seg(x, 1, 2, PAD_ZERO, 0, 0, nullptr);
-    p.w = h->blob + g.w_off;
-    p.bias = h->blob + g.b_off;
-    p.y = out.raw;
-    p.y_elu = out.elu;
-    p.y_bs = (long long)x.L * g.N;
-    p.y_rs = g.N;
-    p.B = B;
-    p.M = x.L;
-    p.N = g.N;
-    p.Ktot = g.Ktot;
+    TapGemmParams p = convtr_params(h, g, x, out, B);
     const int rc = run_tap(h, st, p);
     y->raw = Act{out.raw, (long long)x.L * s * cout, cout, x.L * s, cout, p.amax_out, p.B};
     y->elu = Act{out.elu, (long long)x.L * s * cout, cout, x.L * s, cout, p.amax_out, p.B};
@@ -937,7 +983,7 @@
 }
 
 
-int lstm_fwd(ac_handle* h, hipStream_t st, const LstmPlan& lp, const Act& x, const LstmWs& ws, Out out, int B, Act2* y) {
+int lstm_fwd(ac_handle* h, hipStream_t st, const LstmPlan& lp, const Act& x, const LstmWs& ws, Out out, int B, Act2* y, bool planes_out) {
     const int D = lp.D, T = x.L, L = lp.layers;
     if (D % 64 != 0 || D > 512) return fail(h, AC_EINVAL, "LSTM width %d unsupported (need 64, 128, 256 or 512)", D);
     if (L < 1 || L > 2) return fail(h, AC_EINVAL, "%d LSTM layers unsupported (1 or 2)", L);
@@ -971,6 +1017,8 @@
             x_amax = amax_of(h, st, x.p, x.bs, x.ts, x.L, x.C, B, x.amax_n == B ? x.amax : nullptr);
             if (!x_amax) return fail(h, AC_ESTATE, "out of amax slots (split16.h)");
         }
+        const unsigned* am = amax_plus(h, st, x, 1.0f, B);
+        const bool planes = planes_out && !h->gemm_fp32 && am && out.elu && h->zrow_off && aligned16(out.elu) && D % 32 == 0 && D <= TAP8_ZROW_FLOATS;
         int* poison = reinterpret_cast<int*>(ws.c);
         if (!h->gemm_fp32) HIPCHK(h, hipMemsetAsync(poison, 0x7f, (size_t)B * sizeof(int), st));
         ProfScope ps(h, st, h->gemm_fp32 ? "lstm_persist_kernel" : fuse_in ? "lstm_persist16_kernel<true>" : "lstm_persist16_kernel<false>", 2.0 * T * (double)B * 4 * D * D * (nroles + (fuse_in ? 1 : 0)),
@@ -982,6 +1030,7 @@
             tp.poison = pz;
             tp.yout = out.raw;
             tp.yout_elu = out.elu;
+            tp.yelu_planes = planes ? 1 : 0;
             tp.y_bs = (long long)T * D;
             tp.clip0 = c0;
             tp.B = nb;
@@ -1000,6 +1049,7 @@
             q.skip = x.p;
             q.yout = out.raw;
             q.yout_elu = out.elu;
+            q.yelu_amax = planes ? am : nullptr;
             q.ctl = h->lp_ctl;
             q.gin_ts = B4D;
             q.h_ts = BD;
@@ -1056,9 +1106,9 @@
             tail(c0, q.B, nullptr);
         }
         HIPCHK(h, hipGetLastError());
-        const unsigned* am = amax_plus(h, st, x, 1.0f, B);
         y->raw = Act{out.raw, (long long)T * D, D, T, D, am, B};
         y->elu = Act{out.elu, (long long)T * D, D, T, D, am, B};
+        if (planes) y->elu.zrow = h->blob + h->zrow_off;
         return AC_OK;
     }
     {
@@ -1338,7 +1388,13 @@
         x = y;
         capture(h, st, x.raw, B);
     }
-    rc = lstm_fwd(h, st, h->enc_lstm, x.raw, ws.lstm, Out{dbg ? ws.take() : nullptr, ws.take()}, B, &y);
+    {
+        const Out lo{dbg ? ws.take() : nullptr, ws.take()};
+        const int T = x.raw.L, D = h->enc_lstm.D;
+        const bool pl = conv_planes_ok(h, h->enc_final, Act{lo.elu, (long long)T * D, D, T, D}, c.last_kernel_size, 1, nullptr, Out{feats, nullptr},
+                                       (long long)T * c.hidden_size, c.hidden_size, B);
+        rc = lstm_fwd(h, st, h->enc_lstm, x.raw, ws.lstm, lo, B, &y, pl);
+    }
     if (rc) return rc;
     ws.give(x);
     if (dbg) { capture(h, st, y.raw, B); ws.give(y.raw.p); y.raw.p = nullptr; }
@@ -1362,7 +1418,13 @@
     if (rc) return rc;
     ws.give(zb);
     capture(h, st, x.raw, B);
-    rc = lstm_fwd(h, st, h->dec_lstm, x.raw, ws.lstm, Out{dbg ? ws.take() : nullptr, ws.take()}, B, &y);
+    {
+        const Out lo{dbg ? ws.take() : nullptr, ws.take()};
+        const int T = x.raw.L, D = h->dec_lstm.D;
+        const Act ye{lo.elu, (long long)T * D, D, T, D};
+        const bool pl = !(c.num_ratios == 1 && dec_tail_ok(h, ye)) && convtr_planes_ok(h, h->dec_up[0], ye, c.upsampling_ratios[0], Out{lo.elu, nullptr}, B);
+        rc = lstm_fwd(h, st, h->dec_lstm, x.raw, ws.lstm, lo, B, &y, pl);
+    }
     if (rc) return rc;
     ws.give(x);
     if (dbg) { capture(h, st, y.raw, B); ws.give(y.raw.p); y.raw.p = nullptr; }
diff --git a/audiocodecs_amd/csrc/lstm_persist.h b/audiocodecs_amd/csrc/lstm_persist.h
--- a/audiocodecs_amd/csrc/lstm_persist.h
+++ b/audiocodecs_amd/csrc/lstm_persist.h
@@ -15,6 +15,7 @@
     const float* skip;
     float* yout;
     float* yout_elu;
+    const unsigned* yelu_amax;
     unsigned* ctl;
     long long gin_ts, h_ts, skip_bs, y_bs;
     int B, T;
@@ -47,6 +48,7 @@
     const int* poison;
     float* yout;
     float* yout_elu;
+    int yelu_planes;
     long long y_bs;
     int clip0, B, T, D;
     int xcds_used;
@@ -79,7 +81,7 @@
     const long long o = (long long)(p.clip0 + b) * p.y_bs + (long long)t0 * p.D;
     for (long long i = (long long)blockIdx.y * 256 + threadIdx.x; i < n; i += 256LL * gridDim.y) {
         if (p.yout) p.yout[o + i] = nan;
-        if (p.yout_elu) p.yout_elu[o + i] = nan;
+        if (p.yout_elu) p.yout_elu[o + i] = p.yelu_planes ? __uint_as_float(0x7e007e00u) : nan;
     }
 }
 
diff --git a/audiocodecs_amd/csrc/lstm_persist16.h b/audiocodecs_amd/csrc/lstm_persist16.h
--- a/audiocodecs_amd/csrc/lstm_persist16.h
+++ b/audiocodecs_amd/csrc/lstm_persist16.h
@@ -251,6 +251,8 @@
     }
     const float* skip_row = p.skip + (live ? erow : (long long)p.clip0) * p.skip_bs + eu;
     if (layer == 1) skip_next = skip_row[0];
+    float yscale = 1.f;
+    if (layer == 1 && p.yelu_amax) yscale = s16_pow2(s16_exponent(*amax_at(p.yelu_amax, (int)(live ? erow : (long long)p.clip0))));
     bf16x8 ap[2][2];
     if (layer == 1) load_a(h0b, p.T > 1 ? 1 : 0, ap);
 
@@ -343,7 +345,17 @@
                 const float yv = hn + skipv;
                 const long long o = erow * p.y_bs + (long long)t * D + eu;
                 if (p.yout) p.yout[o] = yv;
-                if (p.yout_elu) p.yout_elu[o] = elu1(yv);
+                if (p.yout_elu) {
+                    const float ye = elu1(yv);
+                    if (p.yelu_amax) {
+                        _Float16* pr = reinterpret_cast<_Float16*>(p.yout_elu) + 2 * (o - eu) + eu;
+                        const _Float16 yh = (_Float16)(ye * yscale);
+                        pr[0] = yh;
+                        pr[D] = (_Float16)__builtin_fmaf(ye, yscale, -(float)yh);
+                    } else {
+                        p.yout_elu[o] = ye;
+                    }
+                }
             }
             const int t1 = t + 1 < p.T ? t + 1 : t;
             if (!ap_ok && !load_valid(h0b, t1, ap)) return false;
diff --git a/audiocodecs_amd/csrc/tap_gemm.h b/audiocodecs_amd/csrc/tap_gemm.h
--- a/audiocodecs_amd/csrc/tap_gemm.h
+++ b/audiocodecs_amd/csrc/tap_gemm.h
@@ -52,6 +52,7 @@
     int amax_rows;
     unsigned* amax_out_rows;
     int epi_direct;
+    const void* a_zrow;
     int stagger;
     unsigned long long* clk;
 };
diff --git a/audiocodecs_amd/csrc/tap_gemm8.h b/audiocodecs_amd/csrc/tap_gemm8.h
--- a/audiocodecs_amd/csrc/tap_gemm8.h
+++ b/audiocodecs_amd/csrc/tap_gemm8.h
@@ -19,6 +19,15 @@
     static constexpr size_t main_bytes = a_bytes + b_bytes;
     static constexpr size_t lds_bytes = main_bytes > C6::epi_bytes ? main_bytes : C6::epi_bytes;
     static_assert(lds_bytes <= 160 * 1024, "one workgroup per CU: slabs + weight ring (or the staged epilogue's tile) within 160 KB of LDS");
+    static constexpr int PL_NBLK = (A_ROWS + 15) / 16;
+    static constexpr int PL_ROWS = PL_NBLK * 16;
+    static constexpr int PL_PLANE = PL_ROWS * 32;
+    static constexpr int APW = (2 * PL_NBLK + 7) / 8;
+    static constexpr size_t pl_slab_bytes = (size_t)2 * PL_PLANE * 2;
+    static constexpr size_t pl_a_bytes = 2 * pl_slab_bytes + 1024;
+    static constexpr size_t pl_main_bytes = pl_a_bytes + b_bytes;
+    static constexpr size_t pl_lds_bytes = pl_main_bytes > C6::epi_bytes ? pl_main_bytes : C6::epi_bytes;
+    static_assert(pl_lds_bytes <= lds_bytes, "the planes-in slabs (64-byte rows) are smaller than the fp32-in ones");
 };
 
 __device__ __forceinline__ void t8_glds16(const void* gsrc, unsigned lds_dst) {
@@ -34,16 +43,18 @@
     asm volatile("s_waitcnt vmcnt(%0)" ::"n"(N) : "memory");
 }
 
-template <int WGM, int WGN, int WMT, int WN, bool RM, bool J1, bool SPREAD = true>
+template <int WGM, int WGN, int WMT, int WN, bool RM, bool J1, bool SPREAD = true, bool PL = false>
 __global__ __launch_bounds__(512, 1) void tap_gemm8_kernel(const TapGemmParams p, const __bf16* __restrict__ wp) {
     using Cfg = Tap8Cfg<WGM, WGN, WMT, WN>;
+    static_assert(!PL || (!RM && !J1), "planes-in: per-clip scale, two or more taps");
+    constexpr int A_PITCH = PL ? 32 : T6_PITCH, A_PLANE = PL ? Cfg::PL_PLANE : Cfg::PLANE;
     constexpr int BM = Cfg::BM, BN = Cfg::BN, NT = Cfg::NT, A_SLOTS = Cfg::A_SLOTS, PLANE = Cfg::PLANE, NTILES = Cfg::NTILES;
     constexpr int HALO = 7;
     unsigned long long clk_t0 = 0, clk_r0 = 0;
     if (p.clk) { clk_t0 = __builtin_amdgcn_s_memtime(); clk_r0 = __builtin_amdgcn_s_memrealtime(); }
     extern __shared__ __attribute__((aligned(16))) float smem[];
     __bf16* As0 = reinterpret_cast<__bf16*>(smem);
-    __bf16* Bs0 = reinterpret_cast<__bf16*>(reinterpret_cast<char*>(smem) + Cfg::a_bytes);
+    __bf16* Bs0 = reinterpret_cast<__bf16*>(reinterpret_cast<char*>(smem) + (PL ? Cfg::pl_a_bytes : Cfg::a_bytes));
     const unsigned bs_lds = (unsigned)(size_t)Bs0;
 
     const int tid = threadIdx.x, lane = tid & 63;
@@ -211,10 +222,12 @@
         t8_glds16(wtile + ((long long)t * ksteps + k0 + ks) * 1024 + pl * 512, bs_lds + (unsigned)((slot * Cfg::B_PIECES + f) * 1024));
     };
 
-    const int a_frag = (wm * WMT * 32 + i32) * T6_PITCH + 8 * kh;
+    const int a_frag = (wm * WMT * 32 + i32) * A_PITCH + (PL ? 0 : 8 * kh);
     auto compute = [&](int abuf, int jr, int slot, auto&& hook) {
-        const __bf16* Ac = As0 + abuf * 2 * PLANE + a_frag + jr * T6_PITCH;
+        const __bf16* Ac = As0 + abuf * 2 * A_PLANE + a_frag + jr * A_PITCH;
         const __bf16* Bc = Bs0 + slot * Cfg::B_SLOT + lane * 8;
+        const int sw0 = PL ? 8 * (kh ^ (((i32 + jr) >> 2) & 3)) : 0;
+        const int a_ks[2] = {PL ? sw0 : 0, PL ? (sw0 ^ 16) : 16};
         f16x8 bf[2][2][WN], af[2][2];
         auto read_b = [&](int ks, f16x8 (&dst)[2][WN]) {
 #pragma unroll
@@ -224,7 +237,7 @@
         };
         auto read_a = [&](int ks, int a, f16x8 (&dst)[2]) {
 #pragma unroll
-            for (int pl = 0; pl < 2; ++pl) dst[pl] = *reinterpret_cast<const f16x8*>(Ac + pl * PLANE + a * 32 * T6_PITCH + ks * 16);
+            for (int pl = 0; pl < 2; ++pl) dst[pl] = *reinterpret_cast<const f16x8*>(Ac + pl * A_PLANE + a * 32 * A_PITCH + a_ks[ks]);
         };
         read_b(0, bf[0]);
         read_a(0, 0, af[0]);
@@ -285,7 +298,86 @@
 #ifdef T6_TRACE
     T6_PHASE(2);
 #endif
-    if constexpr (J1) {
+    if constexpr (PL) {
+        constexpr int APW = Cfg::APW, NBLK = Cfg::PL_NBLK;
+        const unsigned as_lds = (unsigned)(size_t)As0;
+        const char* a_src[APW];
+        unsigned a_dst[APW];
+        {
+            const char* xb = reinterpret_cast<const char*>(sg.x + (long long)b * sg.bs);
+            const char* zb = reinterpret_cast<const char*>(p.a_zrow);
+            const int unit = (lane & 3) ^ ((lane >> 4) & 3);
+#pragma unroll
+            for (int i = 0; i < APW; ++i) {
+                const int tr = wave + 8 * i;
+                const bool real = tr < 2 * NBLK;
+                const int pl = real ? tr / NBLK : 0, blk = tr % NBLK;
+                const int row = blk * 16 + (lane >> 2);
+                const long long jj = real && row < R ? src_index(sg, m0 + row - sg.pad) : -1;
+                a_src[i] = (jj < 0 ? zb : xb + jj * sg.ts * 4) + pl * sg.cin * 2 + unit * 16;
+                a_dst[i] = real ? (unsigned)((pl * A_PLANE + blk * 512) * 2) : (unsigned)(2 * Cfg::pl_slab_bytes);
+            }
+        }
+        auto issue_a_piece = [&](int c, bool live, int slab, int i) {
+            const char* src = live ? a_src[i] + c * (KC * 2) : reinterpret_cast<const char*>(p.a_zrow) + (lane & 3) * 16;
+            const unsigned dst = __builtin_amdgcn_readfirstlane(live ? (unsigned)(slab * Cfg::pl_slab_bytes) + a_dst[i] : (unsigned)(2 * Cfg::pl_slab_bytes));
+            t8_glds16(src, as_lds + dst);
+        };
+        auto issue_a = [&](int c, bool live, int slab) {
+#pragma unroll
+            for (int i = 0; i < APW; ++i) issue_a_piece(c, live, slab, i);
+        };
+        issue_b(0, 0, 0);
+        issue_a(0, true, 0);
+        t8_wait<0>();
+        lds_barrier();
+#ifdef T6_TRACE
+        T6_PHASE(6);
+#endif
+        auto stage = [&](int c, int j, auto issue_tag) {
+            constexpr bool ISSUE = decltype(issue_tag)::value;
+            const int s = c * seg_J + j;
+            int nc = c, nj = j + 1;
+            if (nj == seg_J) { nj = 0; nc = c + 1; }
+            const bool has_next = ISSUE || nc < NC;
+            T8_STAMP(0);
+            if constexpr (SPREAD) {
+                T8_STAMP(1);
+                constexpr int NTASK = Cfg::PPW + (ISSUE ? APW : 0);
+                compute(c & 1, j * rowstep, s & 1, [&](int u) {
+                    const int lo = u * NTASK / UNITS, hi = (u + 1) * NTASK / UNITS;
+#pragma unroll
+                    for (int t = 0; t < NTASK; ++t) {
+                        if (t < lo || t >= hi) continue;
+                        if (t < Cfg::PPW) {
+                            if (has_next) issue_piece(nc, nj, (s + 1) & 1, t);
+                        } else {
+                            issue_a_piece(c + 1, c + 1 < NC, (c + 1) & 1, t - Cfg::PPW);
+                        }
+                    }
+                });
+            } else {
+                if (has_next) issue_b(nc, nj, (s + 1) & 1);
+                if (ISSUE) issue_a(c + 1, c + 1 < NC, (c + 1) & 1);
+                __builtin_amdgcn_sched_barrier(0);
+                T8_STAMP(1);
+                compute(c & 1, j * rowstep, s & 1, no_hook);
+            }
+            __builtin_amdgcn_sched_barrier(0);
+            T8_STAMP(2);
+            if (ISSUE) t8_wait<APW>(); else t8_wait<0>();
+            T8_STAMP(3);
+            lds_barrier();
+            T8_STAMP(4);
+#ifdef T6_TRACE
+            ++t8_stage;
+#endif
+        };
+        for (int c = 0; c < NC; ++c) {
+            stage(c, 0, T{});
+            for (int j = 1; j < seg_J; ++j) stage(c, j, F{});
+        }
+    } else if constexpr (J1) {
         f32x4 raA[A_SLOTS], raB[A_SLOTS];
         issue_b(0, 0, 0);
         load_a(0, true, raA);
diff --git a/audiocodecs_amd/csrc/tap_route.h b/audiocodecs_amd/csrc/tap_route.h
--- a/audiocodecs_amd/csrc/tap_route.h
+++ b/audiocodecs_amd/csrc/tap_route.h
@@ -13,7 +13,7 @@
 
 enum class TapFamily { scalar, vec, tap4, tap6, tap6_dil, tap8 };
 
-enum { TK_RM = 1, TK_J1 = 2, TK_SPREAD = 4 };
+enum { TK_RM = 1, TK_J1 = 2, TK_SPREAD = 4, TK_PL = 8 };
 constexpr int tap_key(int wgm, int wgn, int wm, int wn, int flags = 0) { return flags << 16 | wgm << 12 | wgn << 8 | wm << 4 | wn; }
 
 struct TapRoute {
@@ -22,12 +22,14 @@
     int wgm = 0, wgn = 0, wm = 0, wn = 0;
     int form8 = 0;
     bool rm = false, j1 = false, spread = false;
+    bool planes = false;
+    bool reject_planes = false;
     bool rowmode = false;
     bool rows_out = false;
     bool epi_direct = false;
     bool dil_slab = false;
     char name[48] = "";
-    int key() const { return tap_key(wgm, wgn, wm, wn, (rm ? TK_RM : 0) | (j1 ? TK_J1 : 0) | (spread ? TK_SPREAD : 0)); }
+    int key() const { return tap_key(wgm, wgn, wm, wn, (rm ? TK_RM : 0) | (j1 ? TK_J1 : 0) | (spread ? TK_SPREAD : 0) | (planes ? TK_PL : 0)); }
 };
 
 inline void tap_route_set(TapRoute& r, TapFamily f, int wgm, int wgn, int wm, int wn) {
@@ -72,6 +74,7 @@
         else if (p.N <= 64) tap_route_set(r, f, 2, 2, 2, 2);
         else if (p.N % 96 == 0 && p.N % 128 != 0) tap_route_set(r, f, 2, 2, 4, 3);
         else tap_route_set(r, f, 2, 2, 4, 4);
+        r.reject_planes = p.a_zrow != nullptr;
         return r;
     }
     r.rowmode = in.want_rowmode && in.winv && p.B == 1 && p.nseg == 1 && p.seg[0].J == 1 && p.seg[0].s == 1 && p.seg[0].pad == 0 &&
@@ -116,9 +119,15 @@
             r.j1 = s0.J == 1;
             r.rm = r.j1 && r.rowmode;
             r.spread = dev.tap8_spread == 2 || (dev.tap8_spread == 1 && r.wgm * r.wm * 32 == 128);
+            if (p.a_zrow) {
+                r.planes = !r.rowmode && !r.j1 && s0.s == 1 && s0.dil == 1 && s0.ts == s0.cin && s0.cin % 32 == 0 && s0.amax != nullptr;
+                r.reject_planes = !r.planes;
+                if (r.planes) std::snprintf(r.name, sizeof r.name, "tap_gemm8_kernel<%d, %d, %d, %d, 2, planes>", r.wgm, r.wgn, r.wm, r.wn);
+            }
             return r;
         }
     }
+    r.reject_planes = p.a_zrow != nullptr;
     int pick = 0;
     if (p.N % 256 == 0) {
         const double wg256 = (double)p.B * cdiv(p.M, 128) * (p.N / 256);
```

New measurement: 42260. About the same (-0.1%).
